# owkin/PyDESeq2

Measured on AMD Instinct MI355X. Metric: genes/sec end-to-end deseq2() (size factors->dispersion->IRLS->Wald), higher is better.
Workload: dtype f64

## Files before the change

### include/deseq_hip.h

```cpp
#ifndef DESEQ_HIP_H
#define DESEQ_HIP_H

#include <stddef.h>
#include <stdint.h>

#ifdef __cplusplus
extern "C" {
#endif

#define DSQ_ABI_VERSION 5
#define DSQ_MAX_P 128
#define DSQ_SHRINK_MAX_P 48
#define DSQ_BFGS_MAX_P 12

typedef struct dsq_ctx dsq_ctx;

enum dsq_status {
    DSQ_OK = 0,
    DSQ_ERR_HIP = -1,
    DSQ_ERR_ARG = -2,
    DSQ_ERR_RANGE = -3,
    DSQ_ERR_NOMEM = -4
};

// ... 114 lines not shown
                       const double* d_pinvXt, int ldx, int N, int G, int P, double min_disp, double max_disp,
                       double min_mu, double* d_normed_mean, double* d_mom, double* d_mu);
int dsq_dev_mom(dsq_ctx* ctx, const int32_t* d_y, int ldn, const double* d_sf, const double* d_Xt,
                const double* d_pinvXt, int ldx, int N, int G, int P, double min_disp,
                double max_disp, double* d_normed_mean, double* d_rough, double* d_moments,
                double* d_mom);
int dsq_dev_lin_mu(dsq_ctx* ctx, const int32_t* d_y, int ldn, const double* d_sf,
                   const double* d_Xt, const double* d_pinvXt, int ldx, int N, int G, int P,
                   double min_mu, double* d_mu);
int dsq_dev_alpha_mle(dsq_ctx* ctx, const int32_t* d_y, const double* d_mu, int ldn,
                      const double* d_Xt, int ldx, int N, int G, int P, const double* d_alpha_hat,
                      double min_disp, double max_disp, double prior_disp_var, int cr_reg,
                      int prior_reg, double* d_alpha, uint8_t* d_converged, int32_t* d_nfev,
                      double* d_nll_const, int const_mode);
typedef struct dsq_cells {
    const int32_t* d_cell_of;
    const double* d_Xc;
    const double* d_XX;
    int n_cells;
} dsq_cells;
int dsq_dev_mom_lin_coef(dsq_ctx* ctx, const int32_t* d_y, int ldn, const double* d_sf, const double* d_Xt,
                         const double* d_pinvXt, int ldx, int N, int G, int P, double min_disp, double max_disp,
                         double min_mu, double* d_normed_mean, double* d_mom, double* d_mu, double* d_coef);
int dsq_dev_alpha_mle2(dsq_ctx* ctx, const int32_t* d_y, const double* d_mu, int ldn, const double* d_Xt, int ldx,
                       int N, int G, int P, const double* d_alpha_hat, double min_disp, double max_disp,
                       double prior_disp_var, int cr_reg, int prior_reg, double* d_alpha, uint8_t* d_converged,
                       int32_t* d_nfev, double* d_nll_const, int const_mode, const dsq_cells* cells,
                       const double* d_coef, const double* d_sf, double min_mu);
int dsq_dev_alpha_mle3(dsq_ctx* ctx, const int32_t* d_y, const double* d_mu, int ldn, const double* d_Xt, int ldx,
                       int N, int G, int P, const double* d_alpha_hat, double min_disp, double max_disp,
                       double prior_disp_var, int cr_reg, int prior_reg, double* d_alpha, uint8_t* d_converged,
                       int32_t* d_nfev, double* d_nll_const, int const_mode, const dsq_cells* cells,
                       const double* d_coef, const double* d_sf, double min_mu, const int32_t* d_rows, int n_rows,
                       const int32_t* d_waves, int n_waves, const double* d_cell_mu);
typedef struct dsq_mix dsq_mix;
int dsq_mix_create(dsq_ctx* ctx, const double* design, int N, int P, dsq_mix** out);
void dsq_mix_destroy(dsq_mix* mix);
int dsq_mix_info(const dsq_mix* mix, int* n_slots, int* n_cells, int* n_continuous);
int dsq_mix_slots(const dsq_mix* mix, int32_t* h_slot_of);
int dsq_mix_bind(dsq_ctx* ctx, const uint16_t* d_ys, const uint8_t* d_big, const double* d_mu_slots);
int dsq_mix_bind2(dsq_ctx* ctx, const uint16_t* d_ys, const uint8_t* d_big, const double* d_mu_slots, int G);
int dsq_dev_mix_counts_to_slots(dsq_ctx* ctx, const int32_t* d_y, int ldn, int G, const dsq_mix* mix, uint16_t* d_ys,
                                uint8_t* d_big);
int dsq_dev_mix_mu_slots(dsq_ctx* ctx, const dsq_mix* mix, const double* d_beta, const double* d_sf, int G,
                         double* d_mu_slots);
int dsq_mix_takes_irls(const dsq_mix* mix, int full_rank);
int dsq_mix_launch_count(void);
int dsq_dev_alpha_mle4(dsq_ctx* ctx, const int32_t* d_y, const double* d_mu, int ldn, const double* d_Xt, int ldx,
                       int N, int G, int P, const double* d_alpha_hat, double min_disp, double max_disp,
                       double prior_disp_var, int cr_reg, int prior_reg, double* d_alpha, uint8_t* d_converged,
                       int32_t* d_nfev, double* d_nll_const, int const_mode, const dsq_cells* cells,
                       const double* d_coef, const double* d_sf, double min_mu, const int32_t* d_rows, int n_rows,
                       const int32_t* d_waves, int n_waves, const double* d_cell_mu, const dsq_mix* mix,
                       const double* d_beta);
int dsq_alpha_rows_eligible(int N, int P, int n_cells);
int dsq_alpha_needs_mu(int N, int P, int n_cells);
int dsq_dev_cell_mu(dsq_ctx* ctx, const double* d_beta, const dsq_cells* cells, int G, int P, double* d_cell_mu);
int dsq_dev_alpha_row_split(dsq_ctx* ctx, const int32_t* d_y, int ldn, int N, int G, int32_t* d_flags);
int dsq_dev_robust_disp(dsq_ctx* ctx, const int32_t* d_y, int ldn, const double* d_sf, const int32_t* d_cell_offsets,
                        const int32_t* d_cell_index, int n_cells, int whole, int max_cell, int N, int G,
                        double* d_robust_disp);
int dsq_dev_robust_disp2(dsq_ctx* ctx, const int32_t* d_y, int ldn, const double* d_sf, const int32_t* d_cell_offsets,
                         const int32_t* d_cell_index, int n_cells, int whole, int max_cell, int min_cell, int N, int G,
                         double* d_robust_disp);
int dsq_dev_lfc_fit(dsq_ctx* ctx, const int32_t* d_y, int ldn, const double* d_sf, const double* d_Xt,
                    const double* d_pinvXt, int ldx, int N, int G, int P, int full_rank, const double* d_disp,
                    double min_mu, double beta_tol, double min_beta, double max_beta, int maxiter, double* d_beta,
                    double* d_mu, double* d_hat, uint8_t* d_converged, int32_t* d_iters, const dsq_cells* cells,
                    const double* d_robust_disp, const uint8_t* d_flags, double cutoff, double* d_cooks,
                    uint8_t* d_any_all, uint8_t* d_any_use, uint8_t* d_any_use_nr, uint8_t* d_few_above,
                    const double* h_ridge, const double* h_contrast, double lfc_null, int alt, double* d_pvals,
                    double* d_stats, double* d_se);
int dsq_dev_lfc_fit2(dsq_ctx* ctx, const int32_t* d_y, int ldn, const double* d_sf, const double* d_Xt,
                     const double* d_pinvXt, int ldx, int N, int G, int P, int full_rank, const double* d_disp,
                     double min_mu, double beta_tol, double min_beta, double max_beta, int maxiter, double* d_beta,
                     double* d_mu, double* d_hat, uint8_t* d_converged, int32_t* d_iters, const dsq_cells* cells,
                     const double* d_robust_disp, const uint8_t* d_flags, double cutoff, double* d_cooks,
                     uint8_t* d_any_all, uint8_t* d_any_use, uint8_t* d_any_use_nr, uint8_t* d_few_above,
                     const double* h_ridge, const double* h_contrast, double lfc_null, int alt, double* d_pvals,
                     double* d_stats, double* d_se, const dsq_mix* mix, int cooks_ld);
int dsq_dev_replace_outliers2(dsq_ctx* ctx, const int32_t* d_y, const double* d_cooks, int ldn, const double* d_sf,
                              const uint8_t* d_flags, const int32_t* d_gene_idx, int n_sel, int N, double cutoff,
                              int32_t* d_y_out, uint8_t* d_all_zero, int cooks_ld, const dsq_mix* mix);
int dsq_dev_irls_layers(dsq_ctx* ctx, const int32_t* d_y, int ldn, const double* d_sf, const double* d_Xt, int ldx,
                        int N, int G, int P, const double* d_disp, const double* d_beta, double min_mu, double* d_mu,
                        double* d_hat);
int dsq_side_begin(dsq_ctx* ctx);
int dsq_side_end(dsq_ctx* ctx);
int dsq_side_wait(dsq_ctx* ctx);
int dsq_side_abort(dsq_ctx* ctx);
int dsq_dev_irls(dsq_ctx* ctx, const int32_t* d_y, int ldn, const double* d_sf, const double* d_Xt,
                 const double* d_pinvXt, int ldx, int N, int G, int P, int full_rank,
                 const double* d_disp, double min_mu, double beta_tol, double min_beta,
                 double max_beta, int maxiter, double* d_beta, double* d_mu, double* d_hat,
                 uint8_t* d_converged, int32_t* d_iters);
int dsq_dev_cooks(dsq_ctx* ctx, const int32_t* d_y, int ldn, const double* d_sf, const double* d_mu,
                  const double* d_hat, const int32_t* d_cell_offsets, const int32_t* d_cell_index,
                  int n_cells, int whole, int max_cell, const uint8_t* d_flags, int N, int G, int P,
                  double cutoff, double* d_cooks, double* d_robust_disp, uint8_t* d_any_all,
                  uint8_t* d_any_use, uint8_t* d_any_use_nr, uint8_t* d_few_above);
int dsq_dev_replace_outliers(dsq_ctx* ctx, const int32_t* d_y, const double* d_cooks, int ldn,
                             const double* d_sf, const uint8_t* d_flags, const int32_t* d_gene_idx,
                             int n_sel, int N, double cutoff, int32_t* d_y_out,
                             uint8_t* d_all_zero);
int dsq_dev_wald(dsq_ctx* ctx, const double* d_mu, int ldn, const double* d_sf, const double* d_Xt,
                 int ldx, int N, int G, int P, const double* d_disp, const double* d_beta,
                 const double* h_ridge, const double* h_contrast, double lfc_null, int alt,
                 double* d_pvals, double* d_stats, double* d_se);
int dsq_dev_lrt(dsq_ctx* ctx, const int32_t* d_y, int ldn, const double* d_sf, const double* d_Xt, int ldx, int P,
                const double* d_Xt_reduced, int ldx_reduced, int P_reduced, int N, int G, const double* d_disp,
                const double* d_beta, const double* d_beta_reduced, double* d_stats, double* d_pvals);
int dsq_dev_chisq_sf(dsq_ctx* ctx, const double* d_x, int n, int df, double* d_out);
int dsq_dev_trend_prior(dsq_ctx* ctx, const double* d_disp, const double* d_means, int n, double min_disp,
                        double max_disp, uint8_t* d_keep, double* d_fitted, double* d_work, double* h_coeffs2,
                        int* h_ok, int* h_n_outer, double* h_squared_logres);
int dsq_lfc_fork_begin(dsq_ctx* ctx);
int dsq_lfc_fork_end(dsq_ctx* ctx);
int dsq_lfc_set_part(dsq_ctx* ctx, const uint8_t* d_part, int want, int phase);
int dsq_lfc_takes_parts(int N, int P, const dsq_cells* cells, const dsq_mix* mix, int full_rank);
int dsq_dev_select_dispersions_part(dsq_ctx* ctx, double* d_genewise_raw, double* d_map_raw, const double* d_fitted, int n,
                                    double min_disp, double max_disp, double squared_logres, double* d_disp,
                                    uint8_t* d_outlier, uint8_t* d_map_converged, const uint8_t* d_conv_late, uint8_t* d_part,
                                    int mode, int ready_limit);
int dsq_alpha_set_late_flags(dsq_ctx* ctx, uint8_t* d_conv_late);
int dsq_lfc_prepare(dsq_ctx* ctx, const double* d_sf, int N, const double* h_ridge, const double* h_contrast, int P);
int dsq_dev_trend_eval(dsq_ctx* ctx, const double* d_normed_means, int n, double a0, double a1,
                       double* d_fitted);
int dsq_dev_select_dispersions(dsq_ctx* ctx, double* d_genewise_raw, double* d_map_raw,
                               const double* d_fitted, int n, double min_disp, double max_disp,
                               double squared_logres, double* d_disp, uint8_t* d_outlier);
int dsq_dev_scatter_rows_f64(dsq_ctx* ctx, const double* d_src, const int32_t* d_idx, int n_idx, int width,
                             double* d_dst);
int dsq_dev_mom_raw(dsq_ctx* ctx, const int32_t* d_y, int ldn, const double* d_ones, const double* d_sf,
                    const double* d_Xt, const double* d_pinvXt, int ldx, int N, int G, int P, double min_disp,
                    double max_disp, double* d_normed_mean, double* d_mom);
int dsq_dev_nll_const(dsq_ctx* ctx, const int32_t* d_y, int ldn, int N, int G, const double* d_disp, double* d_cst);
int dsq_dev_nll_scaled(dsq_ctx* ctx, const int32_t* d_y, const double* d_mu, int ldn, int N, int G,
                       const double* d_disp, const double* d_scale, const double* d_cst, double* d_nll);
int dsq_dev_logmeans_poscounts(dsq_ctx* ctx, const int32_t* d_y, int ldn, int N, int G, double* d_logmeans,
                               uint8_t* d_usable);
int dsq_dev_vst(dsq_ctx* ctx, const void* d_counts_sm, int count_type, int N, int G, const double* d_sf, int mode,
                double a0, double a1, double* d_out);
int dsq_inf_lfc_shrink_nbinom_glm2(dsq_ctx* ctx, const void* counts, int count_type, int count_layout,
                                   const double* design, const double* size, const double* offset, int N, int G,
                                   int P, double prior_no_shrink_scale, double prior_scale, int shrink_index,
                                   double* beta_out, double* inv_hessian_out, uint8_t* converged, int optimizer);
int dsq_inf_lfc_shrink_nbinom_glm(dsq_ctx* ctx, const void* counts, int count_type, int count_layout,
                                  const double* design, const double* size, const double* offset, int N, int G,
                                  int P, double prior_no_shrink_scale, double prior_scale, int shrink_index,
                                  double* beta_out, double* inv_hessian_out, uint8_t* converged);
int dsq_dev_lfc_shrink(dsq_ctx* ctx, const int32_t* d_y, int ldn, const double* d_offset, const double* d_Xt,
                       int ldx, int N, int G, int P, const double* d_size, double prior_no_shrink_scale,
                       double prior_scale, int shrink_index, double* d_beta, double* d_inv_hessian,
                       uint8_t* d_converged);
int dsq_dev_lfc_shrink2(dsq_ctx* ctx, const int32_t* d_y, int ldn, const double* d_offset, const double* d_Xt,
                        int ldx, int N, int G, int P, const double* d_size, double prior_no_shrink_scale,
                        double prior_scale, int shrink_index, double* d_beta, double* d_inv_hessian,
                        uint8_t* d_converged, double* d_ih_entry);
int dsq_dev_lfc_shrink3(dsq_ctx* ctx, const int32_t* d_y, int ldn, const double* d_offset, const double* d_Xt,
                        int ldx, int N, int G, int P, const double* d_size, double prior_no_shrink_scale,
                        double prior_scale, int shrink_index, double* d_beta, double* d_inv_hessian,
                        uint8_t* d_converged, double* d_ih_entry, int optimizer);
int dsq_dev_padj_prepare(dsq_ctx* ctx, const double* d_base_mean, const double* d_pvalue, int n, double alpha,
                         unsigned long long* d_sorted_p, int32_t* d_sorted_idx, uint8_t* d_bins,
                         double* h_out200, int* h_n_valid);
int dsq_dev_padj_finish(dsq_ctx* ctx, const unsigned long long* d_sorted_p, const int32_t* d_sorted_idx,
// ... 41 lines not shown
```

### pydeseq2_amd/_lib.py

```python
from __future__ import annotations

import ctypes as C
import os

import numpy as np

_HERE = os.path.dirname(os.path.abspath(__file__))
LIB_PATH = os.environ.get("DSQ_LIB", os.path.join(_HERE, "libdeseq_hip.so"))

DSQ_MAX_P = 128
DSQ_SHRINK_MAX_P = 48
_DEBUG = bool(os.environ.get("DSQ_DEBUG"))
SAMPLE_MAJOR, GENE_MAJOR = 0, 1
I32, I64 = 0, 1
ALT = {None: 0, "greaterAbs": 1, "lessAbs": 2, "greater": 3, "less": 4}

c_void_p, c_int, c_double, c_size_t = C.c_void_p, C.c_int, C.c_double, C.c_size_t
_vp = c_void_p
HOOK_FN = C.CFUNCTYPE(None, c_void_p)


class DsqCells(C.Structure):

    _fields_ = [("d_cell_of", C.c_void_p), ("d_Xc", C.c_void_p), ("d_XX", C.c_void_p), ("n_cells", C.c_int)]
# ... 89 lines not shown
    proto("dsq_dev_select_dispersions", _vp, _vp, _vp, _vp, c_int, c_double, c_double, c_double, _vp, _vp)
    proto("dsq_dev_scatter_rows_f64", _vp, _vp, _vp, c_int, c_int, _vp)
    proto("dsq_dev_sf_keys_compact", _vp, _vp, c_int, c_int, c_int, _vp, _vp, _vp, _vp, C.POINTER(c_int))
    proto("dsq_prior_mad_work_doubles", c_int, res=c_size_t)
    proto("dsq_size_factors_work_doubles", c_int, c_int, res=c_size_t)
    proto("dsq_dev_mom_lin_mu", _vp, _vp, c_int, _vp, _vp, _vp, c_int, c_int, c_int, c_int, c_double, c_double,
          c_double, _vp, _vp, _vp)
    proto("dsq_dev_mom_raw", _vp, _vp, c_int, _vp, _vp, _vp, _vp, c_int, c_int, c_int, c_int, c_double, c_double,
          _vp, _vp)
    proto("dsq_dev_nll_const", _vp, _vp, c_int, c_int, c_int, _vp, _vp)
    proto("dsq_dev_nll_scaled", _vp, _vp, _vp, c_int, c_int, c_int, _vp, _vp, _vp, _vp)
    proto("dsq_dev_logmeans_poscounts", _vp, _vp, c_int, c_int, c_int, _vp, _vp)
    proto("dsq_dev_vst", _vp, _vp, c_int, c_int, c_int, _vp, c_int, c_double, c_double, _vp)
    proto("dsq_inf_lfc_shrink_nbinom_glm2", _vp, _vp, c_int, c_int, _vp, _vp, _vp, c_int, c_int, c_int, c_double,
          c_double, c_int, _vp, _vp, _vp, c_int)
    proto("dsq_inf_lfc_shrink_nbinom_glm", _vp, _vp, c_int, c_int, _vp, _vp, _vp, c_int, c_int, c_int, c_double,
          c_double, c_int, _vp, _vp, _vp)
    proto("dsq_dev_lfc_shrink", _vp, _vp, c_int, _vp, _vp, c_int, c_int, c_int, c_int, _vp, c_double, c_double,
          c_int, _vp, _vp, _vp)
    proto("dsq_dev_lfc_shrink2", _vp, _vp, c_int, _vp, _vp, c_int, c_int, c_int, c_int, _vp, c_double, c_double,
          c_int, _vp, _vp, _vp, _vp)
    proto("dsq_dev_lfc_shrink3", _vp, _vp, c_int, _vp, _vp, c_int, c_int, c_int, c_int, _vp, c_double, c_double,
          c_int, _vp, _vp, _vp, _vp, c_int)
    proto("dsq_dev_padj_prepare", _vp, _vp, _vp, c_int, c_double, _vp, _vp, _vp, _vp, C.POINTER(c_int))
    proto("dsq_dev_padj_finish", _vp, _vp, _vp, _vp, c_int, c_int, c_int, _vp)
    proto("dsq_d2d", _vp, _vp, _vp, c_size_t)
    cells_p = C.POINTER(DsqCells)
    proto("dsq_dev_mom_lin_coef", _vp, _vp, c_int, _vp, _vp, _vp, c_int, c_int, c_int, c_int, c_double, c_double,
          c_double, _vp, _vp, _vp, _vp)
    proto("dsq_dev_alpha_mle2", _vp, _vp, _vp, c_int, _vp, c_int, c_int, c_int, c_int, _vp, c_double, c_double,
          c_double, c_int, c_int, _vp, _vp, _vp, _vp, c_int, cells_p, _vp, _vp, c_double)
    proto("dsq_dev_alpha_mle3", _vp, _vp, _vp, c_int, _vp, c_int, c_int, c_int, c_int, _vp, c_double, c_double,
          c_double, c_int, c_int, _vp, _vp, _vp, _vp, c_int, cells_p, _vp, _vp, c_double, _vp, c_int, _vp, c_int, _vp)
    proto("dsq_dev_alpha_mle4", _vp, _vp, _vp, c_int, _vp, c_int, c_int, c_int, c_int, _vp, c_double, c_double,
          c_double, c_int, c_int, _vp, _vp, _vp, _vp, c_int, cells_p, _vp, _vp, c_double, _vp, c_int, _vp, c_int, _vp,
          _vp, _vp)
    proto("dsq_mix_create", _vp, _vp, c_int, c_int, C.POINTER(_vp))
    proto("dsq_mix_destroy", _vp, res=None)
    proto("dsq_mix_launch_count")
    proto("dsq_mix_slots", _vp, _vp)
    proto("dsq_mix_takes_irls", _vp, c_int)
    proto("dsq_mix_info", _vp, C.POINTER(c_int), C.POINTER(c_int), C.POINTER(c_int))
    proto("dsq_alpha_rows_eligible", c_int, c_int, c_int)
    proto("dsq_alpha_needs_mu", c_int, c_int, c_int)
    proto("dsq_dev_cell_mu", _vp, _vp, cells_p, c_int, c_int, _vp)
    proto("dsq_dev_alpha_row_split", _vp, _vp, c_int, c_int, c_int, _vp)
    proto("dsq_dev_robust_disp", _vp, _vp, c_int, _vp, _vp, _vp, c_int, c_int, c_int, c_int, c_int, _vp)
    proto("dsq_dev_robust_disp2", _vp, _vp, c_int, _vp, _vp, _vp, c_int, c_int, c_int, c_int, c_int, c_int, _vp)
    proto("dsq_dev_lfc_fit", _vp, _vp, c_int, _vp, _vp, _vp, c_int, c_int, c_int, c_int, c_int, _vp, c_double,
          c_double, c_double, c_double, c_int, _vp, _vp, _vp, _vp, _vp, cells_p, _vp, _vp, c_double, _vp, _vp, _vp,
          _vp, _vp, _vp, _vp, c_double, c_int, _vp, _vp, _vp)
    proto("dsq_dev_lfc_fit2", _vp, _vp, c_int, _vp, _vp, _vp, c_int, c_int, c_int, c_int, c_int, _vp, c_double,
          c_double, c_double, c_double, c_int, _vp, _vp, _vp, _vp, _vp, cells_p, _vp, _vp, c_double, _vp, _vp, _vp,
          _vp, _vp, _vp, _vp, c_double, c_int, _vp, _vp, _vp, _vp, c_int)
    proto("dsq_dev_irls_layers", _vp, _vp, c_int, _vp, _vp, c_int, c_int, c_int, c_int, _vp, _vp, c_double, _vp, _vp)
    proto("dsq_side_begin", _vp)
    proto("dsq_side_end", _vp)
    proto("dsq_side_wait", _vp)
    proto("dsq_side_abort", _vp)
    proto("dsq_set_deferred", _vp, c_int)
    proto("dsq_lfc_fork_begin", _vp)
    proto("dsq_lfc_fork_end", _vp)
    proto("dsq_lfc_set_part", _vp, _vp, c_int, c_int)
    proto("dsq_lfc_takes_parts", c_int, c_int, cells_p, _vp, c_int)
    proto("dsq_dev_select_dispersions_part", _vp, _vp, _vp, _vp, c_int, c_double, c_double, c_double, _vp, _vp, _vp, _vp, _vp,
          c_int, c_int)
    proto("dsq_alpha_set_late_flags", _vp, _vp)
    proto("dsq_lfc_prepare", _vp, _vp, c_int, _vp, _vp, c_int)
    proto("dsq_irls_order_hint", _vp, _vp, c_int)
    proto("dsq_set_alpha_hook", _vp, _vp, _vp)
    proto("dsq_upload_counts_i32", _vp, _vp, c_int, c_size_t, _vp, C.POINTER(c_int))
    proto("dsq_host_alloc", _vp, c_size_t, C.POINTER(_vp))
    proto("dsq_host_free", _vp, _vp)
    proto("dsq_d2h_async", _vp, _vp, _vp, c_size_t)
    proto("dsq_h2d_async", _vp, _vp, _vp, c_size_t)
    proto("dsq_dev_alpha_mle", _vp, _vp, _vp, c_int, _vp, c_int, c_int, c_int, c_int, _vp, c_double,
          c_double, c_double, c_int, c_int, _vp, _vp, _vp, _vp, c_int)
    proto("dsq_dev_irls", _vp, _vp, c_int, _vp, _vp, _vp, c_int, c_int, c_int, c_int, c_int, _vp, c_double,
          c_double, c_double, c_double, c_int, _vp, _vp, _vp, _vp, _vp)
    proto("dsq_dev_cooks", _vp, _vp, c_int, _vp, _vp, _vp, _vp, _vp, c_int, c_int, c_int, _vp, c_int, c_int,
          c_int, c_double, _vp, _vp, _vp, _vp, _vp, _vp)
    proto("dsq_dev_replace_outliers", _vp, _vp, _vp, c_int, _vp, _vp, _vp, c_int, c_int, c_double, _vp, _vp)
    proto("dsq_dev_replace_outliers2", _vp, _vp, _vp, c_int, _vp, _vp, _vp, c_int, c_int, c_double, _vp, _vp, c_int, _vp)
    proto("dsq_dev_wald", _vp, _vp, c_int, _vp, _vp, c_int, c_int, c_int, c_int, _vp, _vp, _vp, _vp,
          c_double, c_int, _vp, _vp, _vp)
    proto("dsq_dev_lrt", _vp, _vp, c_int, _vp, _vp, c_int, c_int, _vp, c_int, c_int, c_int, c_int, _vp, _vp, _vp, _vp, _vp)
    proto("dsq_dev_chisq_sf", _vp, _vp, c_int, c_int, _vp)
    proto("dsq_dev_gather_rows_f64", _vp, _vp, c_int, _vp, c_int, c_int, _vp)
    proto("dsq_dev_gather_rows_i32", _vp, _vp, c_int, _vp, c_int, c_int, _vp)
    proto("dsq_comm_unique_id", _vp, C.c_char_p, c_int)
    proto("dsq_comm_init", _vp, C.c_char_p, c_int, c_int)
    proto("dsq_comm_destroy", _vp)
    proto("dsq_comm_allreduce_sum", _vp, _vp, c_size_t, c_int)
    proto("dsq_comm_allgather", _vp, _vp, _vp, c_size_t)
    proto("dsq_dev_sf_keys", _vp, _vp, c_int, c_int, c_int, _vp, _vp, _vp)
    proto("dsq_dev_sf_count", _vp, _vp, c_int, c_int, _vp)
    proto("dsq_dev_sf_init", _vp, _vp, c_int, _vp, _vp)
    proto("dsq_dev_sf_hist", _vp, _vp, c_int, c_int, _vp, c_int, _vp)
    proto("dsq_dev_sf_pick", _vp, _vp, c_int, c_int, _vp, _vp)
    proto("dsq_dev_sf_finish", _vp, _vp, _vp, c_int, _vp)
    _lib = lib
    return lib


EXPORTS = [
    "dsq_create", "dsq_destroy", "dsq_last_error", "dsq_device_info", "dsq_sync", "dsq_debug_pending_error", "dsq_timer_start",
    "dsq_timer_stop", "dsq_last_alpha_kernel", "dsq_malloc", "dsq_free", "dsq_memset", "dsq_h2d", "dsq_d2h", "dsq_h2d_2d",
    "dsq_d2h_2d", "dsq_inf_lin_reg_mu", "dsq_inf_irls", "dsq_inf_alpha_mle", "dsq_inf_wald_test",
    "dsq_inf_fit_rough_dispersions", "dsq_inf_fit_moments_dispersions", "dsq_dev_trend_loss_grad", "dsq_dev_trend_fit", "dsq_dev_prior_mad",
    "dsq_dev_counts_to_gene_major", "dsq_dev_f64_to_gene_major", "dsq_dev_logmeans",
    "dsq_dev_size_factors", "dsq_dev_mom", "dsq_dev_lin_mu", "dsq_dev_alpha_mle", "dsq_dev_irls",
    "dsq_dev_cooks", "dsq_dev_replace_outliers", "dsq_dev_wald", "dsq_dev_gather_rows_f64",
    "dsq_dev_gather_rows_i32", "dsq_comm_unique_id", "dsq_comm_init", "dsq_comm_destroy",
    "dsq_comm_allreduce_sum", "dsq_comm_allgather", "dsq_dev_sf_keys", "dsq_dev_sf_count", "dsq_dev_sf_init",
    "dsq_dev_sf_hist", "dsq_dev_sf_pick", "dsq_dev_sf_finish", "dsq_dev_trend_eval", "dsq_dev_trend_prior", "dsq_dev_select_dispersions",
    "dsq_dev_scatter_rows_f64", "dsq_d2d", "dsq_dev_mom_lin_mu", "dsq_dev_sf_keys_compact", "dsq_prior_mad_work_doubles", "dsq_size_factors_work_doubles", "dsq_dev_mom_raw", "dsq_dev_nll_const", "dsq_dev_nll_scaled", "dsq_dev_logmeans_poscounts", "dsq_dev_vst", "dsq_inf_lfc_shrink_nbinom_glm", "dsq_dev_lfc_shrink", "dsq_dev_lfc_shrink2", "dsq_dev_lfc_shrink3", "dsq_dev_padj_prepare", "dsq_dev_padj_finish", "dsq_host_alloc", "dsq_host_free", "dsq_d2h_async", "dsq_h2d_async",
    "dsq_dev_size_factors_new", "dsq_dev_mom_lin_coef", "dsq_dev_alpha_mle2", "dsq_dev_robust_disp", "dsq_dev_robust_disp2", "dsq_dev_lfc_fit", "dsq_dev_lfc_fit2", "dsq_dev_irls_layers",
    "dsq_side_begin", "dsq_side_end", "dsq_side_wait", "dsq_side_abort", "dsq_set_deferred", "dsq_irls_order_hint", "dsq_set_alpha_hook", "dsq_dev_alpha_mle3", "dsq_dev_alpha_mle4", "dsq_mix_create", "dsq_mix_destroy", "dsq_mix_info", "dsq_mix_slots", "dsq_mix_takes_irls", "dsq_dev_replace_outliers2", "dsq_mix_launch_count", "dsq_alpha_rows_eligible", "dsq_alpha_needs_mu", "dsq_dev_cell_mu", "dsq_dev_alpha_row_split",
    "dsq_upload_counts_i32", "dsq_inf_dispersion_trend_gamma_glm", "dsq_inf_grid_fit_alpha", "dsq_inf_grid_fit_beta",
    "dsq_inf_irls2", "dsq_inf_alpha_mle2", "dsq_inf_lfc_shrink_nbinom_glm2", "dsq_inf_fit_moments_dispersions2",
    "dsq_abi_version", "dsq_plugin_cache_config", "dsq_plugin_cache_clear", "dsq_plugin_cache_stats",
    "dsq_plugin_digest_host", "dsq_comm_info", "dsq_host_sync_count", "dsq_dev_pack2", "dsq_dev_unzip2",
    "dsq_mix_bind", "dsq_mix_bind2", "dsq_dev_mix_counts_to_slots", "dsq_dev_mix_mu_slots",
    "dsq_lfc_fork_begin", "dsq_lfc_fork_end", "dsq_lfc_set_part", "dsq_lfc_takes_parts", "dsq_dev_select_dispersions_part", "dsq_lfc_prepare", "dsq_alpha_set_late_flags",
    "dsq_dev_lrt", "dsq_dev_chisq_sf",
]


def ptr(a):
    if a is None:
        return None
    if isinstance(a, np.ndarray):
        return a.ctypes.data
    return a


class Context:

    def __init__(self, device: int = 0):
        self.lib = load()
        h = _vp()
        rc = self.lib.dsq_create(int(device), C.byref(h))
        if rc != 0 or not h.value:
            raise DsqError(
                f"dsq_create(device={device}) failed (rc={rc}): no usable MI355X / HIP runtime. "
                "pydeseq2_amd runs on the GPU only."
            )
        self.h = h
        self.device = device

    def close(self):
        if getattr(self, "h", None) is not None and self.h.value:
            for bufs in self.__dict__.pop("_padj_buffers", {}).values():
                for b in bufs:
                    b.free()
            self.lib.dsq_destroy(self.h)
            self.h = _vp()

    def __del__(self):
        try:
            self.close()
        except Exception:
            pass

    def call(self, name, *args):
        rc = getattr(self.lib, name)(self.h, *args)
        if _DEBUG:
            pend = self.lib.dsq_debug_pending_error().decode()
            if pend:
                print(f"[dsq debug] pending HIP error after {name}: {pend}", flush=True)
        if rc != 0:
            msg = self.lib.dsq_last_error(self.h).decode(errors="replace")
            if rc == -2:
                raise ValueError(msg)
            raise DsqError(f"{name} failed (rc={rc}): {msg}")

    def device_info(self):
        name, arch = C.create_string_buffer(256), C.create_string_buffer(256)
        cu, mem = c_int(), c_size_t()
        self.call("dsq_device_info", name, 256, C.byref(cu), C.byref(mem), arch, 256)
        return dict(name=name.value.decode(), arch=arch.value.decode(), cu_count=cu.value, mem_bytes=mem.value)

    def sync(self):
        self.call("dsq_sync")

    def timer_start(self):
        self.call("dsq_timer_start")

    def timer_stop(self) -> float:
        ms = C.c_float()
        self.call("dsq_timer_stop", C.byref(ms))
        return float(ms.value)

    def malloc(self, nbytes: int) -> int:
        p = _vp()
        self.call("dsq_malloc", c_size_t(int(nbytes)), C.byref(p))
        return p.value

    def free(self, dptr):
        if dptr:
            self.call("dsq_free", _vp(dptr))

    def memset(self, dptr, value, nbytes):
        self.call("dsq_memset", _vp(dptr), int(value), c_size_t(int(nbytes)))

    def h2d(self, dptr, arr: np.ndarray):
        arr = np.ascontiguousarray(arr)
        self.call("dsq_h2d", _vp(dptr), _vp(arr.ctypes.data), c_size_t(arr.nbytes))
# ... 116 lines not shown
```

### pydeseq2_amd/csrc/dsq_capi_dev.hip

```cpp
#include "dsq_capi_internal.h"

extern "C" {

int dsq_dev_counts_to_gene_major(dsq_ctx* ctx, const void* d_src, int count_type, int layout, int N, int G,
                                 int32_t* d_dst, int ldn, int* h_bad) {
    DSQ_CHECK_ARG(ldn >= N, "ldn < N");
    int* d_bad = (int*)ctx->d_scratch;
    DSQ_HIP(hipMemsetAsync(d_bad, 0, sizeof(int), ctx->stream));
    DSQ_HIP(dsq::launch_transpose_counts(ctx->stream, d_src, count_type, layout, N, G, d_dst, ldn, d_bad));
    if (h_bad) {
        DSQ_HIP(hipMemcpyAsync(h_bad, d_bad, sizeof(int), hipMemcpyDeviceToHost, ctx->stream));
        DSQ_HIP(hipStreamSynchronize(ctx->stream));
    }
    return DSQ_OK;
}

int dsq_dev_f64_to_gene_major(dsq_ctx* ctx, const double* d_src, int layout, int N, int G, double* d_dst,
                              int ldn) {
    DSQ_HIP(dsq::launch_transpose_f64(ctx->stream, d_src, layout, N, G, d_dst, ldn));
    return DSQ_OK;
}

int dsq_dev_logmeans(dsq_ctx* ctx, const int32_t* d_y, int ldn, int N, int G, double* d_logmeans,
                     uint8_t* d_nonzero) {
// ... 442 lines not shown
                     const double* d_pinvXt, int ldx, int N, int G, int P, int full_rank, const double* d_disp,
                     double min_mu, double beta_tol, double min_beta, double max_beta, int maxiter, double* d_beta,
                     double* d_mu, double* d_hat, uint8_t* d_converged, int32_t* d_iters, const dsq_cells* cells,
                     const double* d_robust_disp, const uint8_t* d_flags, double cutoff, double* d_cooks,
                     uint8_t* d_any_all, uint8_t* d_any_use, uint8_t* d_any_use_nr, uint8_t* d_few_above,
                     const double* h_ridge, const double* h_contrast, double lfc_null, int alt, double* d_pvals,
                     double* d_stats, double* d_se, const dsq_mix* mix, int cooks_ld) {
    DSQ_CHECK_ARG(P >= 1 && P <= DSQ_MAX_P, "P out of range");
    DSQ_CHECK_ARG(mix == nullptr || (mix->d.P == P && mix->d.N == N), "mix: built for another design");
    DSQ_CHECK_ARG(cooks_ld == 0 || (mix != nullptr && cooks_ld >= mix->d.Ns && dsq::irls_takes_mix(&mix->d, full_rank)),
                  "cooks_ld: a slot-ordered Cook's layer needs a mixed design the kernel takes and a pitch >= its slots");
    DSQ_CHECK_ARG(cells == nullptr || cells->n_cells <= dsq::kMaxCells, "too many design cells for the cell path");
    DSQ_CHECK_ARG(d_flags == nullptr || (d_robust_disp && d_any_all && d_any_use && d_any_use_nr && d_few_above),
                  "the fused Cook's bookkeeping needs the robust dispersions and the four flag vectors");
    DSQ_CHECK_ARG(h_ridge == nullptr || (h_contrast && d_pvals && d_stats && d_se && alt >= 0 && alt <= 4),
                  "the fused Wald test needs contrast, outputs and a valid alternative");
    if (G <= 0) return DSQ_OK;
    dsq::IrlsExtras ex{};
    ex.cells = to_cells(cells);
    if (mix != nullptr) ex.mix = &mix->d;
    ex.cooks_ld = cooks_ld;
    if (d_flags != nullptr) {
        ex.robust_disp = d_robust_disp; ex.flags = d_flags; ex.cutoff = cutoff; ex.cooks = d_cooks;
        ex.any_all = d_any_all; ex.any_use = d_any_use; ex.any_use_nr = d_any_use_nr; ex.few_above = d_few_above;
    }
    if (h_ridge != nullptr) {
        double* d_ridge;
        double* h_stage;
        { const int rc = ridge_stage(ctx, P, &d_ridge, &h_stage); if (rc != DSQ_OK) return fail(ctx, rc, "ridge staging: out of memory"); }
        double* d_contrast = d_ridge + P * P;
        const bool in_place = ctx->lfc_part != nullptr &&
                              (ctx->lfc_phase == 2 || (ctx->lfc_phase == 1 && ctx->lfc_prepared_wald &&
                                                       ctx->lfc_prepared_N == N && ctx->lfc_prepared_P == P));
        if (!in_place) {
            std::memcpy(h_stage, h_ridge, (size_t)P * P * sizeof(double));
            std::memcpy(h_stage + P * P, h_contrast, (size_t)P * sizeof(double));
            DSQ_HIP(hipMemcpyAsync(d_ridge, h_stage, (size_t)(P * P + P) * sizeof(double), hipMemcpyHostToDevice,
                                   ctx->stream));
        }
        ex.ridge = d_ridge; ex.contrast = d_contrast; ex.lfc_null = lfc_null; ex.alt = alt;
        ex.pvals = d_pvals; ex.stats = d_stats; ex.se = d_se;
    }
    return run_irls(ctx, d_y, ldn, d_sf, d_Xt, d_pinvXt, ldx, N, G, P, full_rank, d_disp, min_mu, beta_tol, min_beta,
                    max_beta, maxiter, d_beta, d_mu, d_hat, d_converged, d_iters, &ex);
}

int dsq_dev_lfc_fit(dsq_ctx* ctx, const int32_t* d_y, int ldn, const double* d_sf, const double* d_Xt,
                    const double* d_pinvXt, int ldx, int N, int G, int P, int full_rank, const double* d_disp,
                    double min_mu, double beta_tol, double min_beta, double max_beta, int maxiter, double* d_beta,
                    double* d_mu, double* d_hat, uint8_t* d_converged, int32_t* d_iters, const dsq_cells* cells,
                    const double* d_robust_disp, const uint8_t* d_flags, double cutoff, double* d_cooks,
                    uint8_t* d_any_all, uint8_t* d_any_use, uint8_t* d_any_use_nr, uint8_t* d_few_above,
                    const double* h_ridge, const double* h_contrast, double lfc_null, int alt, double* d_pvals,
                    double* d_stats, double* d_se) {
    return dsq_dev_lfc_fit2(ctx, d_y, ldn, d_sf, d_Xt, d_pinvXt, ldx, N, G, P, full_rank, d_disp, min_mu, beta_tol,
                            min_beta, max_beta, maxiter, d_beta, d_mu, d_hat, d_converged, d_iters, cells, d_robust_disp,
                            d_flags, cutoff, d_cooks, d_any_all, d_any_use, d_any_use_nr, d_few_above, h_ridge, h_contrast,
                            lfc_null, alt, d_pvals, d_stats, d_se, nullptr, 0);
}

int dsq_dev_cooks(dsq_ctx* ctx, const int32_t* d_y, int ldn, const double* d_sf, const double* d_mu,
                  const double* d_hat, const int32_t* d_cell_offsets, const int32_t* d_cell_index,
                  int n_cells, int whole, int max_cell, const uint8_t* d_flags, int N, int G, int P,
                  double cutoff, double* d_cooks, double* d_robust_disp, uint8_t* d_any_all,
                  uint8_t* d_any_use, uint8_t* d_any_use_nr, uint8_t* d_few_above) {
    DSQ_CHECK_ARG((whole ? N : max_cell) <= 16384, "a design cell with more than 16384 samples is not supported");
    DSQ_HIP(dsq::launch_cooks(ctx->stream, d_y, ldn, d_sf, d_mu, d_hat, d_cell_offsets, d_cell_index,
                              n_cells, whole, max_cell, d_flags, N, G, P, cutoff, d_cooks, d_robust_disp,
                              d_any_all, d_any_use, d_any_use_nr, d_few_above));
    return DSQ_OK;
}

int dsq_dev_replace_outliers2(dsq_ctx* ctx, const int32_t* d_y, const double* d_cooks, int ldn,
                              const double* d_sf, const uint8_t* d_flags, const int32_t* d_gene_idx,
                              int n_sel, int N, double cutoff, int32_t* d_y_out, uint8_t* d_all_zero, int cooks_ld,
                              const dsq_mix* mix) {
    DSQ_CHECK_ARG(cooks_ld == 0 || (mix != nullptr && mix->d.N == N && cooks_ld >= mix->d.Ns),
                  "cooks_ld: a slot-ordered Cook's layer comes with the mixed design that wrote it");
    DSQ_HIP(dsq::launch_replace(ctx->stream, d_y, d_cooks, ldn, d_sf, d_flags, d_gene_idx, n_sel, N, cutoff,
                                d_y_out, d_all_zero, cooks_ld, cooks_ld != 0 ? mix->d.slot_of : nullptr));
    return DSQ_OK;
}

int dsq_dev_replace_outliers(dsq_ctx* ctx, const int32_t* d_y, const double* d_cooks, int ldn,
                             const double* d_sf, const uint8_t* d_flags, const int32_t* d_gene_idx,
                             int n_sel, int N, double cutoff, int32_t* d_y_out, uint8_t* d_all_zero) {
    return dsq_dev_replace_outliers2(ctx, d_y, d_cooks, ldn, d_sf, d_flags, d_gene_idx, n_sel, N, cutoff, d_y_out,
                                     d_all_zero, 0, nullptr);
}

int dsq_dev_wald(dsq_ctx* ctx, const double* d_mu, int ldn, const double* d_sf, const double* d_Xt, int ldx,
                 int N, int G, int P, const double* d_disp, const double* d_beta, const double* h_ridge,
                 const double* h_contrast, double lfc_null, int alt, double* d_pvals, double* d_stats,
                 double* d_se) {
    DSQ_CHECK_ARG(P >= 1 && P <= DSQ_MAX_P, "P out of range");
    DSQ_CHECK_ARG(alt >= 0 && alt <= 4, "unknown alternative hypothesis");
    double* d_ridge;
    double* h_unused;
    { const int rc = ridge_stage(ctx, P, &d_ridge, &h_unused); if (rc != DSQ_OK) return fail(ctx, rc, "ridge staging: out of memory"); }
    double* d_contrast = d_ridge + (P <= 48 ? 48 * 48 : P * P);
    DSQ_HIP(hipMemcpyAsync(d_ridge, h_ridge, (size_t)P * P * sizeof(double), hipMemcpyHostToDevice, ctx->stream));
    DSQ_HIP(hipMemcpyAsync(d_contrast, h_contrast, (size_t)P * sizeof(double), hipMemcpyHostToDevice, ctx->stream));
    DSQ_HIP(hipStreamSynchronize(ctx->stream));
    DSQ_HIP(dsq::launch_wald(ctx->stream, d_mu, ldn, d_sf, d_Xt, ldx, N, G, P, d_disp, d_beta, d_ridge,
                             d_contrast, lfc_null, alt, d_pvals, d_stats, d_se));
    return DSQ_OK;
}

int dsq_dev_lrt(dsq_ctx* ctx, const int32_t* d_y, int ldn, const double* d_sf, const double* d_Xt, int ldx, int P,
                const double* d_Xt_reduced, int ldx_reduced, int P_reduced, int N, int G, const double* d_disp,
                const double* d_beta, const double* d_beta_reduced, double* d_stats, double* d_pvals) {
    DSQ_CHECK_ARG(P >= 2 && P <= DSQ_MAX_P, "P out of range");
    DSQ_CHECK_ARG(P_reduced >= 1 && P_reduced < P, "P_reduced: between 1 and P - 1 columns");
    DSQ_CHECK_ARG(ldn >= N && ldx >= N && ldx_reduced >= N, "a leading dimension is smaller than N");
    DSQ_HIP(dsq::launch_lrt(ctx->stream, d_y, ldn, d_sf, d_Xt, ldx, P, d_Xt_reduced, ldx_reduced, P_reduced, N, G, d_disp,
                            d_beta, d_beta_reduced, d_stats, d_pvals));
    return DSQ_OK;
}

int dsq_dev_chisq_sf(dsq_ctx* ctx, const double* d_x, int n, int df, double* d_out) {
    DSQ_CHECK_ARG(df >= 1 && df <= DSQ_MAX_P - 1, "df: an integer between 1 and 127");
    DSQ_HIP(dsq::launch_chisq_sf(ctx->stream, d_x, n, df, d_out));
    return DSQ_OK;
}

int dsq_dev_gather_rows_f64(dsq_ctx* ctx, const double* d_src, int ld, const int32_t* d_idx, int n_idx,
                            int ncols, double* d_dst) {
    DSQ_HIP(dsq::launch_gather_rows_f64(ctx->stream, d_src, ld, d_idx, n_idx, ncols, d_dst));
    return DSQ_OK;
}

int dsq_dev_lfc_shrink3(dsq_ctx* ctx, const int32_t* d_y, int ldn, const double* d_offset, const double* d_Xt,
                        int ldx, int N, int G, int P, const double* d_size, double prior_no_shrink_scale,
                        double prior_scale, int shrink_index, double* d_beta, double* d_inv_hessian,
                        uint8_t* d_converged, double* d_ih_entry, int optimizer) {
    DSQ_CHECK_ARG(P >= 1 && P <= DSQ_SHRINK_MAX_P, "P out of range (apeGLM shrinkage: at most 48 design columns)");
    DSQ_CHECK_ARG(shrink_index >= 0 && shrink_index < P, "shrink_index out of range");
    DSQ_CHECK_ARG(d_ih_entry == nullptr || P <= DSQ_BFGS_MAX_P, "d_ih_entry: designs of at most 12 columns (wider: d_inv_hessian)");
    DSQ_CHECK_ARG(optimizer >= 0 && optimizer <= 2, "optimizer: 0 (L-BFGS-B), 1 (BFGS) or 2 (Newton-CG)");
    DSQ_CHECK_ARG(optimizer == 0 || P <= DSQ_BFGS_MAX_P, "optimizer BFGS / Newton-CG: designs of at most 12 columns");
    DSQ_HIP(dsq::launch_shrink(ctx->stream, d_y, ldn, d_offset, d_Xt, ldx, N, G, P, d_size, prior_no_shrink_scale,
                               prior_scale, shrink_index, d_beta, d_inv_hessian, d_converged, d_ih_entry, optimizer));
    return DSQ_OK;
}

int dsq_dev_lfc_shrink2(dsq_ctx* ctx, const int32_t* d_y, int ldn, const double* d_offset, const double* d_Xt,
                        int ldx, int N, int G, int P, const double* d_size, double prior_no_shrink_scale,
                        double prior_scale, int shrink_index, double* d_beta, double* d_inv_hessian,
                        uint8_t* d_converged, double* d_ih_entry) {
    return dsq_dev_lfc_shrink3(ctx, d_y, ldn, d_offset, d_Xt, ldx, N, G, P, d_size, prior_no_shrink_scale, prior_scale,
                               shrink_index, d_beta, d_inv_hessian, d_converged, d_ih_entry, 0);
}

int dsq_dev_lfc_shrink(dsq_ctx* ctx, const int32_t* d_y, int ldn, const double* d_offset, const double* d_Xt,
                       int ldx, int N, int G, int P, const double* d_size, double prior_no_shrink_scale,
                       double prior_scale, int shrink_index, double* d_beta, double* d_inv_hessian,
                       uint8_t* d_converged) {
    return dsq_dev_lfc_shrink2(ctx, d_y, ldn, d_offset, d_Xt, ldx, N, G, P, d_size, prior_no_shrink_scale, prior_scale,
                               shrink_index, d_beta, d_inv_hessian, d_converged, nullptr);
}

int dsq_dev_vst(dsq_ctx* ctx, const void* d_counts_sm, int count_type, int N, int G, const double* d_sf, int mode,
                double a0, double a1, double* d_out) {
    DSQ_CHECK_ARG(mode == 0 || mode == 1, "mode: 0 parametric trend, 1 mean dispersion");
    DSQ_HIP(dsq::launch_vst(ctx->stream, d_counts_sm, count_type, N, G, d_sf, mode, a0, a1, d_out));
    return DSQ_OK;
// ... 222 lines not shown
```

### pydeseq2_amd/csrc/dsq_capi_internal.h

```cpp
#pragma once
#include <hip/hip_runtime.h>

#include <dlfcn.h>

#include <algorithm>
#include <cmath>
#include <cstdio>
#include <cstdlib>
#include <cstring>
#include <string>
#include <thread>
#include <vector>

#include <atomic>
#include <mutex>

extern std::atomic<unsigned long long> g_dsq_host_syncs;
#define hipStreamSynchronize(s) (++g_dsq_host_syncs, (hipStreamSynchronize)(s))
#define hipEventSynchronize(e) (++g_dsq_host_syncs, (hipEventSynchronize)(e))

#include "../../include/deseq_hip.h"
#include "dsq_launch.h"
namespace dsq_pc {
struct Cache;
}

struct dsq_mix {
    dsq::MixDesign d{};
    void* d_block = nullptr;
    int device = 0;
};

struct dsq_ctx {
    int device = 0;
    hipStream_t stream = nullptr;
    hipStream_t main_stream = nullptr, side_stream = nullptr;
    hipStream_t small_stream = nullptr;
    hipEvent_t ev_small0 = nullptr, ev_small1 = nullptr;
    hipEvent_t ev_fork = nullptr, ev_join = nullptr;
    hipEvent_t ev0 = nullptr, ev1 = nullptr, evk0 = nullptr, evk1 = nullptr;
    float last_kernel_ms = 0.0f;
    int last_n_grid = 0;
    double* d_scratch = nullptr;
    int32_t* d_counter = nullptr;
    int32_t* d_list = nullptr;
    size_t list_cap = 0;
    void* d_trend_grid = nullptr;
    double* d_lsf = nullptr;
    void* d_sum = nullptr;
    size_t sum_cap = 0, sum_sort_bytes = 0;
    size_t lsf_cap = 0;
    void* stage[2] = {nullptr, nullptr};
    hipEvent_t stage_ev[2] = {nullptr, nullptr};
    void* d_stage16[2] = {nullptr, nullptr};
    const int32_t* d_irls_hint = nullptr;
    int irls_hint_genes = 0;
    void (*alpha_hook)(void*) = nullptr;
    void* alpha_hook_arg = nullptr;
    int deferred = 0;
    int32_t* h_pin = nullptr;
    double* d_ridge_wide = nullptr;
    double* h_ridge_wide = nullptr;
    void* d_ws = nullptr;
    size_t ws_cap = 0;
    void* d_resume = nullptr;
    size_t resume_cap = 0;
    void* d_mix = nullptr;
    size_t mix_cap = 0;
    const uint16_t* bind_ys = nullptr;
    const uint8_t* bind_big = nullptr;
    const double* bind_mu = nullptr;
    int bind_G = 0;
    void* d_mixw = nullptr;
    size_t mixw_cap = 0;
    int32_t* d_redo = nullptr;
    size_t redo_cap = 0;
    hipStream_t lfc_stream = nullptr, lfc_return = nullptr;
    hipEvent_t ev_lfc_fork = nullptr, ev_lfc_done = nullptr, ev_lfc_part = nullptr;
    const uint8_t* lfc_part = nullptr;
    int lfc_want = 0, lfc_phase = 0;
    uint8_t* alpha_conv_late = nullptr;
    int lfc_prepared_N = 0, lfc_prepared_P = 0, lfc_prepared_wald = 0;
    int lfc_pending_G = 0;
    int32_t* d_lfc_aux = nullptr;
    size_t lfc_aux_cap = 0;
    dsq_pc::Cache* pc = nullptr;
    struct PluginDesign* designs = nullptr;
    void* comm = nullptr;
    int comm_rank = 0, comm_world = 1;
    std::string err;
};

void dsq_internal_destroy_plugin(dsq_ctx* ctx);

namespace {
void fire_alpha_hook(void* c) {
    dsq_ctx* ctx = (dsq_ctx*)c;
    if (ctx->alpha_hook == nullptr) return;
    void (*fn)(void*) = ctx->alpha_hook;
    ctx->alpha_hook = nullptr;
    fn(ctx->alpha_hook_arg);
}
}

namespace {

constexpr size_t kScratchBytes = 32 * 1024;
constexpr int kDeferredMaxGenes = 2048;

inline int ridge_stage(dsq_ctx* ctx, int P, double** d, double** h) {
    if (P <= 48) {
        *d = ctx->d_scratch + 1664;
        *h = (double*)(ctx->h_pin + (P <= 32 ? 16 : 4096));
        return DSQ_OK;
    }
    const size_t bytes = (size_t)(DSQ_MAX_P * DSQ_MAX_P + DSQ_MAX_P) * sizeof(double);
    if (ctx->d_ridge_wide == nullptr && hipMalloc((void**)&ctx->d_ridge_wide, bytes) != hipSuccess) {
        ctx->d_ridge_wide = nullptr;
        return DSQ_ERR_NOMEM;
    }
    if (ctx->h_ridge_wide == nullptr && hipHostMalloc((void**)&ctx->h_ridge_wide, bytes, hipHostMallocDefault) != hipSuccess) {
        ctx->h_ridge_wide = nullptr;
        return DSQ_ERR_NOMEM;
    }
    *d = ctx->d_ridge_wide;
    *h = ctx->h_ridge_wide;
    return DSQ_OK;
}

int fail(dsq_ctx* c, int code, const std::string& msg) {
    if (c) {
        c->err = msg;
        c->bind_ys = nullptr;
        c->bind_big = nullptr;
        c->bind_mu = nullptr;
        c->bind_G = 0;
    }
    return code;
}

#define DSQ_HIP(call)                                                                            \
    do {                                                                                         \
        hipError_t e_ = (call);                                                                  \
        if (e_ != hipSuccess)                                                                    \
            return fail(ctx, DSQ_ERR_HIP, std::string(#call) + ": " + hipGetErrorString(e_));    \
    } while (0)

#define DSQ_CHECK_ARG(cond, msg)                          \
    do {                                                  \
        if (!(cond)) return fail(ctx, DSQ_ERR_ARG, msg);  \
    } while (0)

inline int pad16(int n) { return (n + 15) & ~15; }

hipError_t ensure_list(dsq_ctx* c, size_t n) {
    if (n <= c->list_cap) return hipSuccess;
    if (c->d_list) (void)hipFree(c->d_list);
    c->d_list = nullptr;
    c->list_cap = 0;
    hipError_t e = hipMalloc((void**)&c->d_list, n * sizeof(int32_t));
    if (e == hipSuccess) c->list_cap = n;
    return e;
}
// ... 150 lines not shown
                                  prior_var, cr_reg, prior_reg, d_alpha, d_conv, d_nfev, d_cnt, ctx->d_list,
                                  d_nll_const, const_mode, extras, d_cnt + 1));
    }
    DSQ_HIP(hipEventRecord(ctx->evk1, ctx->stream));
    fire_alpha_hook(ctx);
    int32_t* h_cnt = ctx->h_pin + 1;
    const bool deferred = ctx->deferred && G <= kDeferredMaxGenes && optimizer == 0 &&
                          !dsq::alpha_is_wide(P, extras != nullptr ? extras->cells.C : 0);
    const int32_t* n_dev = deferred ? d_cnt : nullptr;
    int32_t n_grid = G;
    if (!deferred) {
        DSQ_HIP(hipMemcpyAsync(h_cnt, d_cnt, sizeof(int32_t), hipMemcpyDeviceToHost, ctx->stream));
        DSQ_HIP(hipStreamSynchronize(ctx->stream));
        DSQ_HIP(hipEventElapsedTime(&ctx->last_kernel_ms, ctx->evk0, ctx->evk1));
        n_grid = *h_cnt;
        ctx->last_n_grid = n_grid;
    } else {
        ctx->last_kernel_ms = -1.0f;
        ctx->last_n_grid = -1;
    }
    if (n_grid > 0) {
        auto up = [](size_t b) { return (b + 255) & ~(size_t)255; };
        const bool from_cells = extras != nullptr && extras->cell_mu != nullptr;
        const bool from_beta = extras != nullptr && extras->mix_beta != nullptr && d_mu == nullptr;
        const bool rebuild = extras != nullptr && (extras->coef != nullptr || from_cells || from_beta);
        const size_t b_work = up((size_t)n_grid * dsq::kAlphaGridWorkDoubles * sizeof(double));
        const size_t b_mu = rebuild ? up((size_t)n_grid * ldn * sizeof(double)) : 0;
        const size_t b_idx = rebuild ? up((size_t)n_grid * sizeof(int32_t)) : 0;
        DSQ_HIP(ensure_ws(ctx, b_work + b_mu + b_idx));
        char* w = (char*)ctx->d_ws;
        double* work = (double*)w;
        if (rebuild) {
            double* musub = (double*)(w + b_work);
            int32_t* idx = (int32_t*)(w + b_work + b_mu);
            if (from_beta)
                DSQ_HIP(dsq::launch_mu_from_beta(ctx->stream, extras->mix_beta, extras->sf, d_Xt, ldx, N, P, ctx->d_list,
                                                 n_grid, musub, ldn, idx, n_dev));
            else if (from_cells)
                DSQ_HIP(dsq::launch_mu_from_cells(ctx->stream, extras->cell_mu, extras->cells.C, extras->sf,
                                                  extras->cells.cell_of, N, ctx->d_list, n_grid, musub, ldn, idx, n_dev));
            else
                DSQ_HIP(dsq::launch_mu_from_coef(ctx->stream, extras->coef, extras->sf, d_Xt, ldx, N, P, extras->min_mu,
                                                 ctx->d_list, n_grid, musub, ldn, idx, n_dev));
            DSQ_HIP(dsq::launch_alpha_grid(ctx->stream, d_y, musub, ldn, d_Xt, ldx, N, P, min_disp, max_disp, d_alpha,
                                           ctx->d_list, n_grid, work, n_dev, true));
        } else {
            DSQ_HIP(dsq::launch_alpha_grid(ctx->stream, d_y, d_mu, ldn, d_Xt, ldx, N, P, min_disp, max_disp, d_alpha,
                                           ctx->d_list, n_grid, work, n_dev));
        }
    }
    return DSQ_OK;
}

}


namespace {
constexpr int kIrlsOrderMinGenes = 1024;
bool irls_order_enabled() {
    static const bool v = getenv("DSQ_NO_IRLS_ORDER") == nullptr;
    return v;
}
}

namespace {
int run_irls(dsq_ctx* ctx, const int32_t* d_y, int ldn, const double* d_sf, const double* d_Xt,
             const double* d_pinvXt, int ldx, int N, int G, int P, int full_rank, const double* d_disp,
             double min_mu, double beta_tol, double min_beta, double max_beta, int maxiter,
             double* d_beta, double* d_mu, double* d_hat, uint8_t* d_converged, int32_t* d_iters,
             const dsq::IrlsExtras* extras, int optimizer = 0) {
    if (G <= 0) return DSQ_OK;
    DSQ_CHECK_ARG(optimizer == 0 || optimizer == 1, "optimizer: 0 (L-BFGS-B) or 1 (BFGS)");
    struct Unbind {
        dsq_ctx* c;
        ~Unbind() { c->bind_ys = nullptr; c->bind_big = nullptr; c->bind_mu = nullptr; c->bind_G = 0; }
    } unbind{ctx};
    if (ctx->bind_G != 0 && ctx->bind_G != G) {
        ctx->bind_ys = nullptr; ctx->bind_big = nullptr; ctx->bind_mu = nullptr; ctx->bind_G = 0;
    }
    dsq::IrlsExtras ex_local{};
    if (extras != nullptr) ex_local = *extras;
    const dsq::MixDesign* const extras_in_mix = ex_local.mix;
    ex_local.optimizer = optimizer;
    DSQ_CHECK_ARG(optimizer == 0 || P <= DSQ_BFGS_MAX_P, "optimizer=\"BFGS\": designs of at most 12 columns");
    extras = &ex_local;
    const uint8_t* const part = ctx->lfc_part;
    const int part_want = ctx->lfc_want, phase = part != nullptr ? ctx->lfc_phase : 0;
    ctx->lfc_part = nullptr; ctx->lfc_phase = 0;
    if (phase != 0) {
        DSQ_CHECK_ARG(phase == 1 || phase == 2, "dsq_lfc_set_part: phase 1 or 2");
        DSQ_CHECK_ARG(optimizer == 0 && !ctx->deferred &&
                          dsq::irls_takes_parts(N, P, ex_local.cells.C, ex_local.mix, full_rank),
                      "a fit in two launches: the default rescue optimiser, not deferred, a design the part-aware kernels take");
        DSQ_CHECK_ARG(phase == 1 ? ctx->lfc_pending_G == 0 : ctx->lfc_pending_G == G,
                      "a fit in two launches: phase 2 follows the phase 1 of the same genes");
        ex_local.part = part;
        ex_local.part_want = part_want;
        ex_local.part_shared_ready = phase == 2 ? 1 : 0;
    }
    const bool ordered = G >= kIrlsOrderMinGenes && dsq::irls_takes_rows(N, P, ex_local.cells.C) && irls_order_enabled();
    const size_t list_ints = (size_t)G * (ordered ? 2 : 1) + (ordered ? (size_t)dsq::irls_order_work_ints() : 0);
    int32_t* fb_list = nullptr;
    int32_t* fb_count = ctx->d_counter;
    if (phase == 1) {
        if (list_ints > ctx->lfc_aux_cap) {
            if (ctx->d_lfc_aux) (void)hipFree(ctx->d_lfc_aux);
            ctx->d_lfc_aux = nullptr; ctx->lfc_aux_cap = 0;
            DSQ_HIP(hipMalloc((void**)&ctx->d_lfc_aux, list_ints * sizeof(int32_t)));
            ctx->lfc_aux_cap = list_ints;
        }
        fb_list = ctx->d_lfc_aux;
        fb_count = ctx->d_counter + 8;
    } else {
        DSQ_HIP(ensure_list(ctx, list_ints));
        fb_list = ctx->d_list;
    }
    if (ordered) {
        int32_t* d_order = fb_list + G;
        DSQ_HIP(dsq::launch_irls_order(ctx->stream, d_disp, ctx->irls_hint_genes == G ? ctx->d_irls_hint : nullptr, G,
                                       d_order, d_order + G));
        ex_local.order = d_order;
    }
    ctx->d_irls_hint = nullptr; ctx->irls_hint_genes = 0;
    const bool prepared = phase == 1 && ctx->lfc_prepared_N == N && ctx->lfc_prepared_P == P;
    ctx->lfc_prepared_N = 0; ctx->lfc_prepared_P = 0; ctx->lfc_prepared_wald = 0;
    if (phase != 2 && !prepared) {
        if ((size_t)N > ctx->lsf_cap) {
            if (ctx->d_lsf) (void)hipFree(ctx->d_lsf);
            ctx->d_lsf = nullptr; ctx->lsf_cap = 0;
            DSQ_HIP(hipMalloc((void**)&ctx->d_lsf, (size_t)N * sizeof(double)));
            ctx->lsf_cap = (size_t)N;
        }
        DSQ_HIP(dsq::launch_log_vec(ctx->stream, d_sf, N, ctx->d_lsf));
    }
    if (!prepared) DSQ_HIP(hipMemsetAsync(fb_count, 0, 2 * sizeof(int32_t), ctx->stream));
    if (ex_local.mix != nullptr && dsq::irls_takes_mix(ex_local.mix, full_rank)) {
        const int n_layers = ((ex_local.flags != nullptr && ex_local.cooks != nullptr) ? 1 : 0) + (d_mu != nullptr ? 1 : 0) +
                             (d_hat != nullptr ? 1 : 0);
        const size_t need = dsq::irls_mix_work_bytes(*ex_local.mix, G, n_layers);
        if (need > ctx->mixw_cap) {
            if (ctx->d_mixw) (void)hipFree(ctx->d_mixw);
            ctx->d_mixw = nullptr; ctx->mixw_cap = 0;
            DSQ_HIP(hipMalloc(&ctx->d_mixw, need));
            ctx->mixw_cap = need;
        }
        ex_local.mix_work = ctx->d_mixw;
        ex_local.mix_work_bytes = ctx->mixw_cap;
        ex_local.mix_queue = fb_count + 1;
        ex_local.mix_ys = ctx->bind_ys;
        ex_local.mix_big = ctx->bind_big;
        if (ex_local.mix_ys == nullptr || ex_local.mix_big == nullptr) {
            const size_t Ns = (size_t)ex_local.mix->Ns;
            const size_t need_s = (size_t)G * Ns * sizeof(uint16_t) + (size_t)G + 256;
            if (need_s > ctx->mix_cap) {
                if (ctx->d_mix) (void)hipFree(ctx->d_mix);
                ctx->d_mix = nullptr; ctx->mix_cap = 0;
                DSQ_HIP(hipMalloc(&ctx->d_mix, need_s));
                ctx->mix_cap = need_s;
            }
            uint16_t* t = (uint16_t*)ctx->d_mix;
            DSQ_HIP(dsq::launch_mix_counts_to_slots(ctx->stream, d_y, ldn, *ex_local.mix, G, t, (uint8_t*)(t + (size_t)G * Ns)));
            ex_local.mix_ys = t;
            ex_local.mix_big = (const uint8_t*)(t + (size_t)G * Ns);
        }
    } else {
        ex_local.mix = nullptr;
// ... 50 lines not shown
```

### pydeseq2_amd/csrc/dsq_k_irls.hip

```cpp
#include <type_traits>

#include "dsq_dispatch.h"
#include "dsq_irls.h"
#include "dsq_launch.h"

namespace dsq {

#if defined(DSQ_PHASE_TIMING)
__device__ unsigned long long g_phase_total_irls[16];
#endif

#ifndef DSQ_IRLS_WAVES_P2
#define DSQ_IRLS_WAVES_P2 4
#endif
constexpr int irls_min_waves(int p) { return p <= 2 ? DSQ_IRLS_WAVES_P2 : (p <= 5 ? 1 : 2); }

template <int P>
__device__ __forceinline__ void epilogue_begin(LfcEpilogue& E, const IrlsExtras& ex, int g, int ldn) {
    if (ex.flags != nullptr) {
        E.flags = ex.flags; E.robust_disp = ex.robust_disp[g]; E.cutoff = ex.cutoff;
        E.cooks_row = ex.cooks ? ex.cooks + (size_t)g * ldn : nullptr;
    }
    if (ex.ridge != nullptr) { E.ridge = ex.ridge; E.contrast = ex.contrast; E.lfc_null = ex.lfc_null; E.alt = ex.alt; }
}
// ... 9 lines not shown

template <int P, int CELL>
__global__ __launch_bounds__(kBlock, CELL == 1 ? cell_min_waves(P) : irls_min_waves(P)) void k_irls(const int32_t* __restrict__ y, int ldn,
                                                 const double* __restrict__ sf, const double* __restrict__ lsf,
                                                 const double* __restrict__ Xt,
                                                 const double* __restrict__ pinvXt, int ldx, int N,
                                                 int G, int full_rank, const double* __restrict__ disp,
                                                 double min_mu, double beta_tol, double min_beta,
                                                 double max_beta, int maxiter, double* __restrict__ beta,
                                                 double* __restrict__ mu, double* __restrict__ hat,
                                                 uint8_t* __restrict__ conv, int32_t* __restrict__ iters,
                                                 int32_t* __restrict__ fb_count,
                                                 int32_t* __restrict__ fb_list, IrlsExtras ex, int stage) {
    __shared__ typename std::conditional<CELL == 1, CellWork<P>, char>::type cellw[kWavesPerBlock];
    extern __shared__ __attribute__((aligned(16))) double irls_lds[];
    const int w = threadIdx.x >> 6;
    const int g = blockIdx.x * kWavesPerBlock + w;
    if (ex.part != nullptr) {
        bool any = false;
#pragma unroll
        for (int k = 0; k < kWavesPerBlock; ++k) {
            const int gk = blockIdx.x * kWavesPerBlock + k;
            any = any || (gk < G && ex.part[gk] == (uint8_t)ex.part_want);
        }
        if (!any) return;
    }
    log_tab_fill();
    double* lds_next = irls_lds;
    if (CELL) {
        constexpr int T = Tri<P>::N;
        double* sXX = lds_next;
        double* sXc = sXX + ex.cells.C * T;
        lds_next = sXc + ex.cells.C * P;
        for (int i = threadIdx.x; i < ex.cells.C * T; i += kBlock) sXX[i] = ex.cells.XX[i];
        for (int i = threadIdx.x; i < ex.cells.C * P; i += kBlock) sXc[i] = ex.cells.Xc[i];
        ex.cells.XX = sXX;
        ex.cells.Xc = sXc;
    }
    const int32_t* yrow = y + (size_t)(g < G ? g : G - 1) * ldn;
    if (stage) {
        const int npad = (N + 15) & ~15;
        double* s_sf = lds_next;
        double* s_lsf = s_sf + npad;
        int32_t* s_cell = (int32_t*)(s_lsf + npad);
        int32_t* s_y = s_cell + npad + (size_t)w * npad;
        for (int n = threadIdx.x; n < N; n += kBlock) {
            s_sf[n] = sf[n];
            s_lsf[n] = lsf != nullptr ? lsf[n] : 0.0;
            if (CELL) s_cell[n] = ex.cells.cell_of[n];
        }
        for (int n = threadIdx.x & 63; n < N; n += 64) s_y[n] = yrow[n];
        sf = s_sf;
        if (lsf != nullptr) lsf = s_lsf;
        if (CELL) ex.cells.cell_of = s_cell;
        yrow = s_y;
    }
    __syncthreads();
    if (g >= G) return;
    if (ex.part != nullptr && ex.part[g] != (uint8_t)ex.part_want) return;
#if defined(DSQ_PHASE_TIMING)
    if ((threadIdx.x & 63) == 0) {
        for (int k = 0; k < kPhases; ++k) g_ph_acc[w][k] = 0;
        g_ph_last[w] = clock64();
        g_ph_cur[w] = 0;
    }
#endif
    IrlsArgs A;
    A.y = yrow; A.sf = sf; A.lsf = lsf; A.Xt = Xt; A.pinvXt = pinvXt; A.ldx = ldx; A.N = N;
    A.disp = disp[g]; A.min_mu = min_mu; A.beta_tol = beta_tol; A.min_beta = min_beta;
    A.max_beta = max_beta; A.maxiter = maxiter; A.full_rank = full_rank != 0;
    if (CELL) { A.cells = &ex.cells; A.cell_ws = CELL == 1 ? (void*)&cellw[w] : nullptr; }
    LfcEpilogue E;
    epilogue_begin<P>(E, ex, g, ldn);
    double b[P];
    const IrlsOut o = irls_gene<DeviceWave, P, CELL>(A, b, mu ? mu + (size_t)g * ldn : nullptr,
                                                     hat ? hat + (size_t)g * ldn : nullptr, &E);
    if ((threadIdx.x & 63) == 0) {
#pragma unroll
        for (int j = 0; j < P; ++j) beta[(size_t)g * P + j] = b[j];
        conv[g] = (uint8_t)o.converged;
        if (iters != nullptr) iters[g] = o.iters;
        if (o.fallback) fb_list[atomicAdd(fb_count, 1)] = g;
        else epilogue_store(E, ex, g);
    }
#if defined(DSQ_PHASE_TIMING)
    DSQ_PHASE(0);
    if ((threadIdx.x & 63) == 0)
        for (int k = 0; k < kPhases; ++k) atomicAdd(&g_phase_total_irls[k], (unsigned long long)g_ph_acc[w][k]);
#endif
}

constexpr int kRowGenes = kBlock / 16;
template <int P>
__global__ __launch_bounds__(kBlock, 2) void k_irls_row(const int32_t* __restrict__ y, int ldn,
                                                        const double* __restrict__ sf, const double* __restrict__ lsf,
                                                        const double* __restrict__ Xt,
                                                        const double* __restrict__ pinvXt, int ldx, int N, int G,
                                                        int full_rank, const double* __restrict__ disp, double min_mu,
                                                        double beta_tol, double min_beta, double max_beta, int maxiter,
                                                        double* __restrict__ beta, double* __restrict__ mu,
                                                        double* __restrict__ hat, uint8_t* __restrict__ conv,
                                                        int32_t* __restrict__ iters, int32_t* __restrict__ fb_count,
                                                        int32_t* __restrict__ fb_list, IrlsExtras ex) {
    __shared__ CellWork<P> cellw[kRowGenes];
    extern __shared__ __attribute__((aligned(16))) double irls_lds[];
    constexpr int T = Tri<P>::N;
    const int row = threadIdx.x >> 4;
    const int slot = blockIdx.x * kRowGenes + row;
    int g = slot < G ? (ex.order != nullptr ? ex.order[slot] : slot) : G;
    if (ex.part != nullptr && g < G && ex.part[g] != (uint8_t)ex.part_want) g = G;
    if (ex.part != nullptr && __syncthreads_count(g < G) == 0) return;
    log_tab_fill();
    double* sXX = irls_lds;
    double* sXc = sXX + ex.cells.C * T;
    const int npad = (N + 15) & ~15;
    double* s_sf = sXc + ex.cells.C * P;
    double* s_lsf = s_sf + npad;
    double* s_pinvc = s_lsf + npad;
    int32_t* s_cell = (int32_t*)(s_pinvc + ex.cells.C * P);
    int32_t* s_rep = s_cell + npad;
    for (int i = threadIdx.x; i < ex.cells.C * T; i += kBlock) sXX[i] = ex.cells.XX[i];
    for (int i = threadIdx.x; i < ex.cells.C * P; i += kBlock) sXc[i] = ex.cells.Xc[i];
    if (full_rank) {
        for (int i = threadIdx.x; i < ex.cells.C; i += kBlock) s_rep[i] = 0x7fffffff;
        __syncthreads();
    }
    for (int n = threadIdx.x; n < N; n += kBlock) {
        s_sf[n] = sf[n];
        s_lsf[n] = lsf != nullptr ? lsf[n] : 0.0;
        const int c = ex.cells.cell_of[n];
        s_cell[n] = c;
        if (full_rank) atomicMin(&s_rep[c], n);
    }
    if (full_rank) {
        __syncthreads();
        for (int i = threadIdx.x; i < ex.cells.C * P; i += kBlock) s_pinvc[i] = pinvXt[(i % P) * ldx + s_rep[i / P]];
    }
    ex.cells.XX = sXX;
    ex.cells.Xc = sXc;
    ex.cells.cell_of = s_cell;
    __syncthreads();
    if (g >= G) return;
    IrlsArgs A;
    A.y = y + (size_t)g * ldn; A.sf = s_sf; A.lsf = lsf != nullptr ? s_lsf : nullptr; A.Xt = Xt; A.pinvXt = pinvXt;
    A.ldx = ldx; A.N = N;
    A.disp = disp[g]; A.min_mu = min_mu; A.beta_tol = beta_tol; A.min_beta = min_beta;
    A.max_beta = max_beta; A.maxiter = maxiter; A.full_rank = full_rank != 0;
    A.cells = &ex.cells;
    A.cell_ws = (void*)&cellw[row];
    A.pinvc = full_rank ? s_pinvc : nullptr;
#if defined(DSQ_PHASE_TIMING)
    if ((threadIdx.x & 63) == 0) {
        for (int k = 0; k < kPhases; ++k) g_ph_acc[threadIdx.x >> 6][k] = 0;
        g_ph_last[threadIdx.x >> 6] = clock64();
        g_ph_cur[threadIdx.x >> 6] = 0;
    }
#endif
    LfcEpilogue E;
    epilogue_begin<P>(E, ex, g, ldn);
    double b[P];
    const IrlsOut o = irls_gene<RowWave, P, 1>(A, b, mu ? mu + (size_t)g * ldn : nullptr,
                                               hat ? hat + (size_t)g * ldn : nullptr, &E);
    if ((threadIdx.x & 15) == 0) {
#pragma unroll
        for (int j = 0; j < P; ++j) beta[(size_t)g * P + j] = b[j];
        conv[g] = (uint8_t)o.converged;
// ... 100 lines not shown
    const int g = fb_list[k];
    IrlsArgs A;
    A.y = y + (size_t)g * ldn; A.sf = sf; A.lsf = lsf; A.Xt = Xt; A.pinvXt = pinvXt; A.ldx = ldx; A.N = N;
    A.disp = disp[g]; A.min_mu = min_mu; A.beta_tol = beta_tol; A.min_beta = min_beta;
    A.max_beta = max_beta; A.maxiter = maxiter; A.full_rank = full_rank != 0;
    __shared__ IrlsRescueWork<P> work[kWavesPerBlock];
    LfcEpilogue E;
    epilogue_begin<P>(E, ex, g, ldn);
    if (ex.cooks_ld != 0 && E.cooks_row != nullptr) E.cooks_row = ex.cooks_tmp + (size_t)k * ldn;
    double b[P];
    const IrlsOut o = irls_rescue_gene<DeviceWave, P>(A, work[threadIdx.x >> 6], b,
                                                      mu ? mu + (size_t)g * ldn : nullptr,
                                                      hat ? hat + (size_t)g * ldn : nullptr, &E, ex.optimizer);
    if ((threadIdx.x & 63) == 0) {
#pragma unroll
        for (int j = 0; j < P; ++j) beta[(size_t)g * P + j] = b[j];
        conv[g] = (uint8_t)o.converged;
        if (iters != nullptr) iters[g] = o.iters;
        epilogue_store(E, ex, g);
    }
}

__global__ __launch_bounds__(kBlock) void k_grid_beta(const int32_t* __restrict__ y, int ldn,
                                                      const double* __restrict__ sf, const double* __restrict__ Xt,
                                                      int ldx, int N, int G, const double* __restrict__ disp,
                                                      double min_mu, double min_beta, double max_beta, int grid_length,
                                                      double* __restrict__ beta) {
    const int g = blockIdx.x * kWavesPerBlock + (threadIdx.x >> 6);
    if (g >= G) return;
    IrlsArgs A;
    A.y = y + (size_t)g * ldn; A.sf = sf; A.lsf = nullptr; A.Xt = Xt; A.pinvXt = nullptr; A.ldx = ldx; A.N = N;
    A.disp = disp[g]; A.min_mu = min_mu; A.beta_tol = 0.0; A.min_beta = min_beta; A.max_beta = max_beta;
    A.maxiter = 0; A.full_rank = false;
    const double a = 1.0 / A.disp;
    double c = 0.0;
    for (int n = DeviceWave::lane(); n < N; n += 64) {
        const double yv = (double)A.y[n];
        c += lgamma_pos(yv + a) - lgamma_pos(yv + 1.0);
    }
    const double cst = DeviceWave::sum(c) - N * lgamma_pos(a);
    double b[2];
    grid_fit_beta2<DeviceWave>(A, a, cst, b, grid_length);
    if ((threadIdx.x & 63) == 0) { beta[2 * g] = b[0]; beta[2 * g + 1] = b[1]; }
}

hipError_t launch_grid_beta(hipStream_t st, const int32_t* y, int ldn, const double* sf, const double* Xt, int ldx,
                            int N, int G, const double* disp, double min_mu, double min_beta, double max_beta,
                            int grid_length, double* beta) {
    if (G <= 0) return hipSuccess;
    hipLaunchKernelGGL(k_grid_beta, dim3(genes_to_blocks(G)), dim3(kBlock), 0, st, y, ldn, sf, Xt, ldx, N, G, disp,
                       min_mu, min_beta, max_beta, grid_length, beta);
    return hipGetLastError();
}

template <int P>
__global__ __launch_bounds__(kBlock) void k_irls_layers(const int32_t* __restrict__ y, int ldn,
                                                        const double* __restrict__ sf, const double* __restrict__ Xt,
                                                        int ldx, int N, int G, const double* __restrict__ disp,
                                                        const double* __restrict__ beta, double min_mu,
                                                        double* __restrict__ mu, double* __restrict__ hat) {
    log_tab_fill();
    __syncthreads();
    const int g = blockIdx.x * kWavesPerBlock + (threadIdx.x >> 6);
    if (g >= G) return;
    IrlsArgs A;
    A.y = y + (size_t)g * ldn; A.sf = sf; A.lsf = nullptr; A.Xt = Xt; A.pinvXt = nullptr; A.ldx = ldx; A.N = N;
    A.disp = disp[g]; A.min_mu = min_mu; A.beta_tol = 0.0; A.min_beta = 0.0; A.max_beta = 0.0; A.maxiter = 0;
    A.full_rank = false;
    double b[P], M[Tri<P>::N], r[P], S;
#pragma unroll
    for (int j = 0; j < P; ++j) b[j] = beta[(size_t)g * P + j];
    irls_sweep<DeviceWave, P>(A, b, 1.0 / A.disp, S, M, r);
    irls_finish<DeviceWave, P>(A, b, M, mu ? mu + (size_t)g * ldn : nullptr, hat ? hat + (size_t)g * ldn : nullptr);
}

hipError_t launch_irls_layers(hipStream_t st, const int32_t* y, int ldn, const double* sf, const double* Xt, int ldx,
                              int N, int G, int P_, const double* disp, const double* beta, double min_mu, double* mu,
                              double* hat) {
    if (G <= 0) return hipSuccess;
    if (P_ > DSQ_REG_MAX_P)
        return launch_wide_irls_layers(st, y, ldn, sf, Xt, ldx, N, G, P_, disp, beta, min_mu, mu, hat);
    DSQ_DISPATCH_P(P_, hipLaunchKernelGGL(k_irls_layers<P>, dim3(genes_to_blocks(G)), dim3(kBlock), 0, st, y, ldn, sf,
                                          Xt, ldx, N, G, disp, beta, min_mu, mu, hat))
    return hipGetLastError();
}

constexpr int kRowMinP = 3;
static bool row_wave_enabled() {
    static const bool v = getenv("DSQ_NO_ROW_WAVE") == nullptr;
    return v;
}
static int row_min_p() {
    static const int v = getenv("DSQ_ROW_MIN_P") ? atoi(getenv("DSQ_ROW_MIN_P")) : 5;
    return v;
}
static size_t row_lds_bytes(int C, int P, int N) {
    const int npad = (N + 15) & ~15;
    return (size_t)C * (P * (P + 1) / 2 + 2 * P) * sizeof(double) + (size_t)npad * 20 + (size_t)kMaxCells * 4;
}

static int irls_row_min_genes() {
    const char* e = getenv("DSQ_IRLS_ROW_MIN_G");
    return e ? atoi(e) : 1024;
}

bool irls_takes_parts(int N, int P_, int n_cells, const MixDesign* mix, int full_rank) {
    (void)N;
    if (mix != nullptr && irls_takes_mix(mix, full_rank)) return true;
    return !(P_ > DSQ_REG_MAX_P || (P_ >= wide_min_p() && (n_cells == 0 || wide_with_cells())));
}

bool irls_takes_rows(int N, int P_, int n_cells) {
    if (P_ > DSQ_REG_MAX_P || (P_ >= wide_min_p() && (n_cells == 0 || wide_with_cells()))) return false;
    return n_cells > kSmallCells && P_ >= kRowMinP && P_ >= row_min_p() && row_wave_enabled() &&
           row_lds_bytes(n_cells, P_, N) <= 40 * 1024;
}

#define DSQ_MIXI_DECL(Q_)                                                                                             \
    bool irls_mix_fits_q##Q_(int Ns, int P);                                                                          \
    void irls_mix_grid_q##Q_(int Ns, int P, int G, int* blocks, int* nw);                                             \
    hipError_t launch_irls_mix_q##Q_(hipStream_t, const int32_t*, int, const uint16_t*, const uint8_t*, const MixDesign&, \
                                     const double*, int, int32_t*, const double*, double, double, double, int, double*, \
                                     double*, double*, uint8_t*, int32_t*, int32_t*, int32_t*, const IrlsExtras&, void*, \
                                     size_t);
DSQ_MIXI_DECL(1)
DSQ_MIXI_DECL(2)
DSQ_MIXI_DECL(3)
#undef DSQ_MIXI_DECL

bool irls_takes_mix(const MixDesign* mix, int full_rank) {
    static const bool off = getenv("DSQ_NO_IRLS_MIX") != nullptr;
    if (off || mix == nullptr || !full_rank || mix->Ginv == nullptr || !alpha_mix_enabled()) return false;
    switch (mix->Q) {
        case 1: return irls_mix_fits_q1(mix->Ns, mix->P);
        case 2: return irls_mix_fits_q2(mix->Ns, mix->P);
        case 3: return irls_mix_fits_q3(mix->Ns, mix->P);
        default: return false;
    }
}

size_t irls_mix_work_bytes(const MixDesign& D, int G, int n_layers) {
    int blocks = 0, nw = 0;
    if (D.Q == 1) irls_mix_grid_q1(D.Ns, D.P, G, &blocks, &nw);
    else if (D.Q == 2) irls_mix_grid_q2(D.Ns, D.P, G, &blocks, &nw);
    else if (D.Q == 3) irls_mix_grid_q3(D.Ns, D.P, G, &blocks, &nw);
    (void)blocks; (void)nw; (void)n_layers;
    return (((size_t)D.Ns * 17 + 63) & ~(size_t)63) + (size_t)(G > 0 ? G : 0) * (kMixMaxP * (kMixMaxP + 1) / 2) * sizeof(double) + 64;
}

static hipError_t launch_irls_mix(hipStream_t st, const int32_t* y, int ldn, const MixDesign& D, const double* sf, int G,
                                  int32_t* queue, const double* disp, double min_mu, double beta_tol, double max_beta,
                                  int maxiter, double* beta, double* mu, double* hat, uint8_t* conv, int32_t* iters,
                                  int32_t* fb_count, int32_t* fb_list, const IrlsExtras& ex, void* work,
                                  size_t work_bytes) {
    switch (D.Q) {
        case 1: return launch_irls_mix_q1(st, y, ldn, ex.mix_ys, ex.mix_big, D, sf, G, queue, disp, min_mu, beta_tol, max_beta, maxiter, beta, mu,
                                          hat, conv, iters, fb_count, fb_list, ex, work, work_bytes);
        case 2: return launch_irls_mix_q2(st, y, ldn, ex.mix_ys, ex.mix_big, D, sf, G, queue, disp, min_mu, beta_tol, max_beta, maxiter, beta, mu,
                                          hat, conv, iters, fb_count, fb_list, ex, work, work_bytes);
        case 3: return launch_irls_mix_q3(st, y, ldn, ex.mix_ys, ex.mix_big, D, sf, G, queue, disp, min_mu, beta_tol, max_beta, maxiter, beta, mu,
                                          hat, conv, iters, fb_count, fb_list, ex, work, work_bytes);
        default: return hipErrorInvalidValue;
    }
}

hipError_t launch_irls(hipStream_t st, const int32_t* y, int ldn, const double* sf, const double* lsf,
// ... 127 lines not shown
```

### pydeseq2_amd/csrc/dsq_k_stats.hip

```cpp
#include <cfloat>
#include <hip/hip_cooperative_groups.h>

#include <cstdio>

#include "dsq_dispatch.h"
#include "dsq_launch.h"
#include "dsq_stats.h"
#include "dsq_trend.h"

namespace dsq {

struct LdsSorter {
    __device__ __forceinline__ static void wave_sync() {
        __builtin_amdgcn_fence(__ATOMIC_RELEASE, "wavefront");
        __builtin_amdgcn_wave_barrier();
        __builtin_amdgcn_fence(__ATOMIC_ACQUIRE, "wavefront");
    }
    __device__ __forceinline__ int operator()(double* buf, int n) const {
        int L = 1;
        while (L < n) L <<= 1;
        const int lane = threadIdx.x & 63;
        for (int k = n + lane; k < L; k += 64) buf[k] = INFINITY;
        wave_sync();
        for (int k = 2; k <= L; k <<= 1) {
// ... 1049 lines not shown
                                                               const double* __restrict__ sf,
                                                               const int32_t* __restrict__ cell_offsets,
                                                               const int32_t* __restrict__ cell_index, int n_cells,
                                                               int whole, int N, int G,
                                                               double* __restrict__ robust_disp,
                                                               int32_t* __restrict__ redo_count,
                                                               int32_t* __restrict__ redo_list, int can_redo) {
    __shared__ BucketWork W[WPB];
    const int w = threadIdx.x >> 6;
    const int g = blockIdx.x * WPB + w;
    if (g >= G) return;
    CellPlan C{cell_offsets, cell_index, n_cells, whole};
    bool failed;
    const double ar = robust_disp_gene_lean<DeviceWave>(y + (size_t)g * ldn, sf, C, N, W[w], failed);
    if ((threadIdx.x & 63) == 0) {
        if (failed && can_redo) redo_list[atomicAdd(redo_count, 1)] = g;
        else robust_disp[g] = failed ? NAN : ar;
    }
}

bool robust_disp_lean_eligible(int min_cell, int max_cell, int whole, int N) {
    const bool off = getenv("DSQ_NO_ROBUST_LEAN") != nullptr;
    const char* mn = getenv("DSQ_ROBUST_LEAN_MIN");
    const int min_big = mn != nullptr ? atoi(mn) : 2048;
    return !off && (whole ? N : min_cell) >= kTrimBucketMin && (whole ? N : max_cell) >= min_big;
}

hipError_t launch_robust_disp(hipStream_t st, const int32_t* y, int ldn, const double* sf,
                              const int32_t* cell_offsets, const int32_t* cell_index, int n_cells, int whole,
                              int max_cell, int N, int G, double* robust_disp, int min_cell, int32_t* redo) {
    if (G <= 0) return hipSuccess;
    const int biggest = whole ? N : max_cell;
    static const bool seg_off = getenv("DSQ_NO_SEG_CELLS") != nullptr;
    const int seg_len = (!whole && !seg_off && biggest <= kSegMaxCell) ? next_pow2(biggest < 2 ? 2 : biggest) : 0;
    const int cap = seg_len > 0 ? kSegBatch + kSegBatch / 2 : trim_cap(biggest);
    const int stride = cap + trim_work_doubles(biggest);
    const size_t per_wave = (size_t)stride * sizeof(double);
    const bool big = biggest >= kTrimBucketMin;
    const bool buffered_fits = per_wave <= 160 * 1024;
    if (!buffered_fits && redo == nullptr) return hipErrorInvalidValue;
    const bool lean = redo != nullptr && (!buffered_fits || robust_disp_lean_eligible(min_cell, max_cell, whole, N));
    if (lean) {
        hipError_t e = hipMemsetAsync(redo, 0, sizeof(int32_t), st);
        if (e != hipSuccess) return e;
        constexpr int WPB = 4;
        hipLaunchKernelGGL((k_robust_disp_lean<WPB>), dim3((G + WPB - 1) / WPB), dim3(64 * WPB), 0, st, y, ldn, sf,
                           cell_offsets, cell_index, n_cells, whole, N, G, robust_disp, redo, redo + 1,
                           buffered_fits ? 1 : 0);
        e = hipGetLastError();
        if (e != hipSuccess || !buffered_fits) return e;
    }
    const int32_t* list = lean ? redo + 1 : nullptr;
    const int32_t* n_dev = lean ? redo : nullptr;
#define DSQ_RD_LAUNCH(WPB) \
    do { if (big) DSQ_RD_LAUNCH_(WPB, true); else DSQ_RD_LAUNCH_(WPB, false); } while (0)
#define DSQ_RD_LAUNCH_(WPB, BIG)                                                                             \
    do {                                                                                                     \
        if (per_wave * WPB > 48 * 1024) {                                                                    \
            (void)hipFuncSetAttribute((const void*)k_robust_disp<WPB, BIG>, hipFuncAttributeMaxDynamicSharedMemorySize, \
                                      (int)(per_wave * WPB));                                                \
            (void)hipGetLastError();                                                                         \
        }                                                                                                    \
        hipLaunchKernelGGL((k_robust_disp<WPB, BIG>), dim3((G + WPB - 1) / WPB), dim3(64 * WPB), per_wave * WPB, st, y, \
                           ldn, sf, cell_offsets, cell_index, n_cells, whole, cap, stride, seg_len, N, G, robust_disp, \
                           list, n_dev);                                                                     \
    } while (0)
    if (per_wave * 4 <= 64 * 1024) DSQ_RD_LAUNCH(4);
    else if (per_wave * 2 <= 160 * 1024) DSQ_RD_LAUNCH(2);
    else DSQ_RD_LAUNCH(1);
#undef DSQ_RD_LAUNCH
#undef DSQ_RD_LAUNCH_
    return hipGetLastError();
}

template <int WPB>
__global__ __launch_bounds__(64 * WPB) void k_replace(const int32_t* __restrict__ y,
                                                      const double* __restrict__ cooks, int ldn,
                                                      const double* __restrict__ sf,
                                                      const uint8_t* __restrict__ flags,
                                                      const int32_t* __restrict__ gene_idx, int n_sel,
                                                      int N, int cap, int stride, double cutoff,
                                                      int32_t* __restrict__ y_out,
                                                      uint8_t* __restrict__ all_zero, int cooks_ld,
                                                      const int32_t* __restrict__ slot_of) {
    extern __shared__ __attribute__((aligned(16))) double lds[];
    const int w = threadIdx.x >> 6;
    const int k = blockIdx.x * WPB + w;
    if (k >= n_sel) return;
    const int g = gene_idx[k];
    const int32_t* yr = y + (size_t)g * ldn;
    const double* ck = cooks + (size_t)g * (slot_of != nullptr ? (size_t)cooks_ld : (size_t)ldn);
    double* scratch = lds + (size_t)w * stride;
    const double tbm = trimmed_base_mean<DeviceWave>(yr, sf, N, 0.2, scratch, LdsSorter(),
                                                     stride > cap ? (BucketWork*)(scratch + cap) : nullptr);
    int nonzero = 0;
    for (int n = DeviceWave::lane(); n < N; n += 64) {
        int v = yr[n];
        if ((flags[n] & 2) && ck[slot_of != nullptr ? slot_of[n] : n] > cutoff) v = (int)(tbm * sf[n]);
        y_out[(size_t)k * ldn + n] = v;
        nonzero |= (v != 0);
    }
    nonzero = DeviceWave::sumi(nonzero);
    if ((threadIdx.x & 63) == 0) all_zero[k] = (uint8_t)(nonzero == 0);
    if (nonzero == 0)
        for (int n = DeviceWave::lane(); n < N; n += 64) y_out[(size_t)k * ldn + n] = yr[n];
}

template <int WPB>
__global__ __launch_bounds__(64 * WPB) void k_replace_lean(const int32_t* __restrict__ y,
                                                           const double* __restrict__ cooks, int ldn,
                                                           const double* __restrict__ sf,
                                                           const uint8_t* __restrict__ flags,
                                                           const int32_t* __restrict__ gene_idx, int n_sel, int N,
                                                           double cutoff, int32_t* __restrict__ y_out,
                                                           uint8_t* __restrict__ all_zero, int cooks_ld,
                                                           const int32_t* __restrict__ slot_of) {
    __shared__ BucketWork W[WPB];
    const int w = threadIdx.x >> 6;
    const int k = blockIdx.x * WPB + w;
    if (k >= n_sel) return;
    const int g = gene_idx[k];
    const int32_t* yr = y + (size_t)g * ldn;
    const double* ck = cooks + (size_t)g * (slot_of != nullptr ? (size_t)cooks_ld : (size_t)ldn);
    bool failed;
    const double tbm = trimmed_base_mean_lean<DeviceWave>(yr, sf, N, 0.2, W[w], failed);
    int nonzero = 0;
    for (int n = DeviceWave::lane(); n < N; n += 64) {
        int v = yr[n];
        if ((flags[n] & 2) && ck[slot_of != nullptr ? slot_of[n] : n] > cutoff) v = (int)(tbm * sf[n]);
        y_out[(size_t)k * ldn + n] = v;
        nonzero |= (v != 0);
    }
    nonzero = DeviceWave::sumi(nonzero);
    if ((threadIdx.x & 63) == 0) all_zero[k] = (uint8_t)(nonzero == 0);
    if (nonzero == 0)
        for (int n = DeviceWave::lane(); n < N; n += 64) y_out[(size_t)k * ldn + n] = yr[n];
}

hipError_t launch_replace(hipStream_t st, const int32_t* y, const double* cooks, int ldn,
                          const double* sf, const uint8_t* flags, const int32_t* gene_idx, int n_sel,
                          int N, double cutoff, int32_t* y_out, uint8_t* all_zero, int cooks_ld,
                          const int32_t* slot_of) {
    if (n_sel <= 0) return hipSuccess;
    const int cap = next_pow2(N);
    const int stride = cap + trim_work_doubles(N);
    const size_t per_wave = (size_t)stride * sizeof(double);
    static const bool force_lean = getenv("DSQ_REPLACE_LEAN") != nullptr;
    if (per_wave > 160 * 1024 || force_lean) {
        constexpr int WPB = 4;
        hipLaunchKernelGGL(k_replace_lean<WPB>, dim3((n_sel + WPB - 1) / WPB), dim3(64 * WPB), 0, st, y, cooks, ldn, sf,
                           flags, gene_idx, n_sel, N, cutoff, y_out, all_zero, cooks_ld, slot_of);
        return hipGetLastError();
    }
#define DSQ_REPL_LAUNCH(WPB)                                                                         \
    do {                                                                                             \
        if (per_wave * WPB > 48 * 1024) {                                                            \
            (void)hipFuncSetAttribute((const void*)k_replace<WPB>, hipFuncAttributeMaxDynamicSharedMemorySize, \
                                      (int)(per_wave * WPB));                                        \
            (void)hipGetLastError();                                                                 \
        }                                                                                            \
        hipLaunchKernelGGL(k_replace<WPB>, dim3((n_sel + WPB - 1) / WPB), dim3(64 * WPB),            \
                           per_wave * WPB, st, y, cooks, ldn, sf, flags, gene_idx, n_sel, N, cap,    \
                           stride, cutoff, y_out, all_zero, cooks_ld, slot_of);                      \
    } while (0)
    if (per_wave * 4 <= 64 * 1024) DSQ_REPL_LAUNCH(4);
    else if (per_wave * 2 <= 160 * 1024) DSQ_REPL_LAUNCH(2);
    else DSQ_REPL_LAUNCH(1);
#undef DSQ_REPL_LAUNCH
    return hipGetLastError();
}

template <class T>
__global__ __launch_bounds__(256) void k_gather_rows(const T* __restrict__ src, int ld,
                                                     const int32_t* __restrict__ idx, int n_idx,
                                                     int ncols, T* __restrict__ dst,
                                                     const int32_t* __restrict__ n_dev = nullptr) {
    const int k = blockIdx.x;
    if (n_dev != nullptr && k >= *n_dev) return;
    const int g = idx[k];
    for (int c = blockIdx.y * 256 + threadIdx.x; c < ncols; c += gridDim.y * 256)
        dst[(size_t)k * ld + c] = src[(size_t)g * ld + c];
}

hipError_t launch_gather_rows_f64(hipStream_t st, const double* src, int ld, const int32_t* idx,
                                  int n_idx, int ncols, double* dst) {
    if (n_idx <= 0) return hipSuccess;
    const int gx = (ncols + 255) / 256 > 64 ? 64 : (ncols + 255) / 256;
    hipLaunchKernelGGL(k_gather_rows<double>, dim3(n_idx, gx), dim3(256), 0, st, src, ld, idx, n_idx, ncols,
                       dst);
    return hipGetLastError();
}

hipError_t launch_gather_rows_i32(hipStream_t st, const int32_t* src, int ld, const int32_t* idx,
                                  int n_idx, int ncols, int32_t* dst, const int32_t* n_dev) {
    if (n_idx <= 0) return hipSuccess;
    const int gx = (ncols + 255) / 256 > 64 ? 64 : (ncols + 255) / 256;
    hipLaunchKernelGGL(k_gather_rows<int32_t>, dim3(n_idx, gx), dim3(256), 0, st, src, ld, idx, n_idx,
                       ncols, dst, n_dev);
    return hipGetLastError();
}

__global__ void k_trend_eval(const double* __restrict__ nm, int n, double a0, double a1,
                             double* __restrict__ fitted) {
    const int i = blockIdx.x * blockDim.x + threadIdx.x;
    if (i < n) fitted[i] = (a1 == 0.0) ? a0 : a0 + a1 / nm[i];
}

__global__ void k_trend_eval_dev(const double* __restrict__ nm, int n, const double* __restrict__ coef,
                                 double* __restrict__ fitted) {
    const int i = blockIdx.x * blockDim.x + threadIdx.x;
    const double a0 = coef[0], a1 = coef[1];
    if (i < n) fitted[i] = (a1 == 0.0) ? a0 : a0 + a1 / nm[i];
}

__global__ void k_select_disp(double* __restrict__ gw_raw, double* __restrict__ map_raw,
                              const double* __restrict__ fitted, int n, double min_disp, double max_disp,
                              double two_sd, double* __restrict__ disp, uint8_t* __restrict__ outlier) {
    const int i = blockIdx.x * blockDim.x + threadIdx.x;
    if (i >= n) return;
    const double gw = fmin(fmax(gw_raw[i], min_disp), max_disp);
    const double mp = fmin(fmax(map_raw[i], min_disp), max_disp);
    const bool out = log(gw) > log(fitted[i]) + two_sd;
    disp[i] = out ? gw : mp;
    outlier[i] = out ? 1 : 0;
    if (gw_raw[i] == gw_raw[i]) gw_raw[i] = gw;
    if (map_raw[i] == map_raw[i]) map_raw[i] = mp;
}

__global__ void k_select_disp_part(double* __restrict__ gw_raw, double* __restrict__ map_raw,
                                   const double* __restrict__ fitted, int n, double min_disp, double max_disp,
                                   double two_sd, double* __restrict__ disp, uint8_t* __restrict__ outlier,
                                   uint8_t* __restrict__ map_conv, const uint8_t* __restrict__ conv_late,
                                   uint8_t* __restrict__ part, int mode, int ready_limit) {
    const int i = blockIdx.x * blockDim.x + threadIdx.x;
    if (i >= n) return;
    if (mode == 1) {
        const bool ready = map_conv[i] == 1 && i < ready_limit;
        part[i] = ready ? 1 : 0;
        if (!ready) return;
    } else {
        if (part[i] != 0) return;
        if (conv_late != nullptr && conv_late[i] != 0xFF) map_conv[i] = conv_late[i];
    }
    const double gw = fmin(fmax(gw_raw[i], min_disp), max_disp);
    const double mp = fmin(fmax(map_raw[i], min_disp), max_disp);
    const bool out = log(gw) > log(fitted[i]) + two_sd;
// ... 635 lines not shown
```

### pydeseq2_amd/csrc/dsq_launch.h

```cpp
#pragma once
#include <hip/hip_runtime.h>

#include <cstdint>

#include "../../include/deseq_hip.h"
#include "dsq_linalg.h"
#include "dsq_mix.h"

namespace dsq {

constexpr int kWavesPerBlock = 4;
constexpr int kBlock = 64 * kWavesPerBlock;

inline int genes_to_blocks(int G) { return (G + kWavesPerBlock - 1) / kWavesPerBlock; }

inline int current_device_cus() {
    static int cache[64] = {0};
    int dev = 0;
    if (hipGetDevice(&dev) != hipSuccess) return 0;
    if (dev >= 0 && dev < 64 && cache[dev] > 0) return cache[dev];
    hipDeviceProp_t prop;
    if (hipGetDeviceProperties(&prop, dev) != hipSuccess) return 0;
    if (dev >= 0 && dev < 64) cache[dev] = prop.multiProcessorCount;
    return prop.multiProcessorCount;
// ... 95 lines not shown
    const uint16_t* mix_ys;
    const double* mix_mu;
};
constexpr int kAlphaEvalCap = 8;
size_t alpha_resume_bytes(int G);
constexpr int kRowTail = 512;
bool alpha_rows_eligible(int N, int P, int n_cells, bool has_coef, int cr_reg);
hipError_t launch_alpha_rows(hipStream_t st, const int32_t* y, int ldn, int N, const int32_t* list, int n_list,
                             int32_t* queue, const double* coef, const double* sf, const CellDesign& cells, int P,
                             double min_mu, const double* alpha_hat, double min_disp, double max_disp, double prior_var,
                             int cr_reg, int prior_reg, double* alpha, uint8_t* conv, int32_t* nfev, int32_t* grid_count,
                             int32_t* grid_list, double* nll_const, int const_mode, int eval_cap, void* park_state,
                             int32_t* park_count, int32_t* park_list);
hipError_t launch_count_big(hipStream_t st, const int32_t* y, int ldn, int N, int G, int32_t* out);
int alpha_rowsc_tail(int N, int P, int n_cells);
hipError_t launch_alpha_rows_c(hipStream_t st, const int32_t* y, int ldn, int N, const int32_t* list, int n_list,
                               int32_t* queue, const double* coef, const double* cell_mu, const double* sf,
                               const CellDesign& cells, int P, double min_mu, const double* alpha_hat, double min_disp,
                               double max_disp, double prior_var, int prior_reg, double* alpha, uint8_t* conv,
                               int32_t* nfev, int32_t* grid_count, int32_t* grid_list, double* nll_const,
                               int const_mode, int eval_cap, void* park_state, int32_t* park_count,
                               int32_t* park_list);
hipError_t launch_cell_mu(hipStream_t st, const double* beta, const double* Xc, int C, int G, int P, double* cell_mu);
hipError_t launch_mu_from_cells(hipStream_t st, const double* cell_mu, int C, const double* sf, const int32_t* cell_of,
                                int N, const int32_t* list, int n_list, double* dst, int ldn, int32_t* idx_out,
                                const int32_t* n_dev = nullptr);
bool alpha_mix_enabled();
int alpha_mix_launches();
bool alpha_mix_fits(const MixDesign& D);
hipError_t launch_alpha_mix(hipStream_t st, const uint16_t* ys, const double* mu_s, const MixDesign& D, const int32_t* list,
                            int n_list, const int32_t* n_dev, int32_t* queue, const double* alpha_hat, double min_disp,
                            double max_disp, double prior_var, int prior_reg, double* alpha, uint8_t* conv, int32_t* nfev,
                            int32_t* grid_count, int32_t* grid_list, double* nll_const, int const_mode, int eval_cap,
                            int resume, void* park_state, int32_t* park_count, int32_t* park_list);
hipError_t launch_mu_from_beta(hipStream_t st, const double* beta, const double* sf, const double* Xt, int ldx, int N,
                               int P, const int32_t* list, int n_list, double* dst, int ldn, int32_t* idx_out,
                               const int32_t* n_dev = nullptr);
bool alpha_wg_eligible(int N);
hipError_t launch_alpha_wg(hipStream_t st, const int32_t* y, int ldn, int N, const int32_t* list, const int32_t* n_dev,
                           int n_cap, const double* coef, const double* sf, const CellDesign& cells, int P,
                           double min_mu, const double* alpha_hat, double prior_var, int prior_reg, double* alpha,
                           uint8_t* conv, int32_t* nfev, int32_t* grid_count, int32_t* grid_list,
                           const double* nll_const, const void* park_state);
hipError_t launch_alpha_bfgs(hipStream_t st, const int32_t* y, const double* mu, int ldn, const double* Xt, int ldx,
                             int N, int G, int P, const double* alpha_hat, double min_disp, double max_disp,
                             double prior_var, int cr_reg, int prior_reg, double* alpha, uint8_t* conv,
                             int32_t* nfev, int32_t* grid_count, int32_t* grid_list);
hipError_t launch_alpha(hipStream_t st, const int32_t* y, const double* mu, int ldn, const double* Xt,
                        int ldx, int N, int G, int P, const double* alpha_hat, double min_disp,
                        double max_disp, double prior_var, int cr_reg, int prior_reg, double* alpha,
                        uint8_t* conv, int32_t* nfev, int32_t* grid_count, int32_t* grid_list,
                        double* nll_const, int const_mode, const AlphaExtras* extras = nullptr, int32_t* queue = nullptr);
hipError_t launch_alpha_grid(hipStream_t st, const int32_t* y, const double* mu, int ldn, const double* Xt,
                             int ldx, int N, int P, double min_disp, double max_disp, double* alpha,
                             const int32_t* grid_list, int n_grid, double* work, const int32_t* n_dev = nullptr,
                             bool mu_compact = false);
constexpr int kAlphaGridWorkDoubles = 103;

struct IrlsExtras {
    CellDesign cells;
    const double* robust_disp;
    const uint8_t* flags;
    double cutoff;
    double* cooks;
    int cooks_ld;
    double* cooks_tmp;
    uint8_t *any_all, *any_use, *any_use_nr, *few_above;
    const double* ridge;
    const double* contrast;
    double lfc_null;
    int alt;
    double *pvals, *stats, *se;
    int optimizer;
    const int32_t* order;
    const MixDesign* mix;
    void* mix_work;
    size_t mix_work_bytes;
    int32_t* mix_queue;
    const uint16_t* mix_ys;
    const uint8_t* mix_big;
    const uint8_t* part;
    int part_want;
    int part_shared_ready;
};
bool irls_takes_parts(int N, int P, int n_cells, const MixDesign* mix, int full_rank);
bool irls_takes_mix(const MixDesign* mix, int full_rank);
size_t irls_mix_work_bytes(const MixDesign& D, int G, int n_layers);
hipError_t launch_replace(hipStream_t st, const int32_t* y, const double* cooks, int ldn,
                          const double* sf, const uint8_t* flags, const int32_t* gene_idx, int n_sel,
                          int N, double cutoff, int32_t* y_out, uint8_t* all_zero, int cooks_ld,
                          const int32_t* slot_of);
bool irls_takes_rows(int N, int P, int n_cells);
hipError_t launch_irls_order(hipStream_t st, const double* disp, const int32_t* hint_iters, int G, int32_t* order,
                             int32_t* work);
int irls_order_work_ints();
hipError_t launch_irls(hipStream_t st, const int32_t* y, int ldn, const double* sf, const double* lsf,
                       const double* Xt,
                       const double* pinvXt, int ldx, int N, int G, int P, int full_rank,
                       const double* disp, double min_mu, double beta_tol, double min_beta,
                       double max_beta, int maxiter, double* beta, double* mu, double* hat,
                       uint8_t* conv, int32_t* iters, int32_t* fb_count, int32_t* fb_list,
                       const IrlsExtras* extras = nullptr);
hipError_t launch_irls_rescue(hipStream_t st, const int32_t* y, int ldn, const double* sf,
                              const double* lsf, const double* Xt, const double* pinvXt, int ldx, int N, int P,
                              int full_rank, const double* disp, double min_mu, double beta_tol,
                              double min_beta, double max_beta, int maxiter, double* beta, double* mu,
                              double* hat, uint8_t* conv, int32_t* iters, const int32_t* fb_list,
                              int n_fb, const IrlsExtras* extras = nullptr, const int32_t* n_dev = nullptr);

bool irls_is_wide(int P, int n_cells);
bool alpha_is_wide(int P, int n_cells);
bool alpha_needs_mu(int N, int P, int n_cells);

hipError_t launch_widen_u16(hipStream_t st, const uint16_t* src, int32_t* dst, size_t n);
hipError_t launch_transpose_counts(hipStream_t st, const void* src, int count_type, int layout, int N,
                                   int G, int32_t* dst, int ldn, int* bad_flag);
hipError_t launch_transpose_f64(hipStream_t st, const double* src, int layout, int N, int G,
                                double* dst, int ldn);
hipError_t launch_logmeans(hipStream_t st, const int32_t* y, int ldn, int N, int G, double* logmeans,
                           uint8_t* nonzero);
hipError_t launch_size_factors(hipStream_t st, const void* counts_sm, int count_type, int N, int G,
                               const double* logmeans, const uint8_t* gene_mask, double* work,
                               double* sf, int zeros_low = 0);
hipError_t launch_mom(hipStream_t st, const int32_t* y, int ldn, const double* sf, const double* Xt,
                      const double* pinvXt, int ldx, int N, int G, int P, double min_disp,
                      double max_disp, double* normed_mean, double* rough, double* moments,
                      double* mom, double* d_scalar, const double* sf_moments = nullptr);
hipError_t launch_mom_lin_mu(hipStream_t st, const int32_t* y, int ldn, const double* sf, const double* Xt,
                             const double* pinvXt, int ldx, int N, int G, int P, double min_disp, double max_disp,
                             double min_mu, double* normed_mean, double* mom, double* mu, double* d_scalar,
                             double* coef = nullptr);
hipError_t launch_mu_from_coef(hipStream_t st, const double* coef, const double* sf, const double* Xt, int ldx, int N,
                               int P, double min_mu, const int32_t* list, int n_list, double* dst, int ldn,
                               int32_t* idx_out, const int32_t* n_dev = nullptr);
hipError_t launch_irls_layers(hipStream_t st, const int32_t* y, int ldn, const double* sf, const double* Xt, int ldx,
                              int N, int G, int P, const double* disp, const double* beta, double min_mu, double* mu,
                              double* hat);
hipError_t launch_nll_const(hipStream_t st, const int32_t* y, int ldn, int N, int G, const double* disp, double* cst);
hipError_t launch_nll_scaled(hipStream_t st, const int32_t* y, const double* mu, int ldn, int N, int G,
                             const double* disp, const double* scale, const double* cst, double* nll);
hipError_t launch_lin_mu(hipStream_t st, const int32_t* y, int ldn, const double* sf, const double* Xt,
                         const double* pinvXt, int ldx, int N, int G, int P, double min_mu,
                         double* mu);
hipError_t launch_wald(hipStream_t st, const double* mu, int ldn, const double* sf, const double* Xt,
                       int ldx, int N, int G, int P, const double* disp, const double* beta,
                       const double* d_ridge, const double* d_contrast, double lfc_null, int alt,
                       double* pvals, double* stats, double* se);
hipError_t launch_lrt(hipStream_t st, const int32_t* y, int ldn, const double* sf, const double* Xf, int ldf, int Pf,
                      const double* Xr, int ldr, int Pr, int N, int G, const double* disp, const double* beta_f,
                      const double* beta_r, double* stat, double* pval);
hipError_t launch_chisq_sf(hipStream_t st, const double* x, int n, int df, double* out);
hipError_t launch_cooks(hipStream_t st, const int32_t* y, int ldn, const double* sf, const double* mu,
                        const double* hat, const int32_t* cell_offsets, const int32_t* cell_index,
                        int n_cells, int whole, int max_cell, const uint8_t* flags, int N, int G,
                        int P, double cutoff, double* cooks, double* robust_disp, uint8_t* any_all,
                        uint8_t* any_use, uint8_t* any_use_nr, uint8_t* few_above);
hipError_t launch_robust_disp(hipStream_t st, const int32_t* y, int ldn, const double* sf,
                              const int32_t* cell_offsets, const int32_t* cell_index, int n_cells, int whole,
                              int max_cell, int N, int G, double* robust_disp, int min_cell = 0, int32_t* redo = nullptr);
hipError_t launch_gather_rows_f64(hipStream_t st, const double* src, int ld, const int32_t* idx,
                                  int n_idx, int ncols, double* dst);
hipError_t launch_shrink(hipStream_t st, const int32_t* y, int ldn, const double* offset, const double* Xt, int ldx,
                         int N, int G, int P, const double* size, double sigma0, double sigma, int shrink_index,
                         double* beta, double* invh, uint8_t* conv, double* ih_entry = nullptr, int optimizer = 0);
size_t summary_sort_temp_bytes(int n);
hipError_t launch_padj_prepare(hipStream_t st, const double* base_mean, const double* pvalue, int n, double alpha,
                               void* sort_tmp, size_t sort_tmp_bytes, void* work, unsigned long long* sorted_p,
                               int* sorted_idx, unsigned char* bins, double* out200, int* counters);
hipError_t launch_padj_numrej(hipStream_t st, const unsigned long long* sorted_p, const int* sorted_idx,
                              const unsigned char* bins, int n_valid, double alpha, double* out200);
hipError_t launch_padj_finish(hipStream_t st, const unsigned long long* sorted_p, const int* sorted_idx,
                              const unsigned char* bins, int n, int n_valid, int j, int* rank_tmp, double* padj);
hipError_t launch_logmeans_pos(hipStream_t st, const int32_t* y, int ldn, int N, int G, double* logmeans,
                               uint8_t* usable);
// ... 58 lines not shown
```

### pydeseq2_amd/pipeline.py

```python
from __future__ import annotations

import os
import time
import warnings
from dataclasses import dataclass, field

import numpy as np
from scipy.stats import f as f_dist

from . import trend as _trend
from ._design import DesignPack, pad16
from ._lib import ALT, HOOK_FN, I32, I64, SAMPLE_MAJOR, Context, DeviceArray, DsqCells, _PinnedPool, _PinnedSlab

import ctypes as C
import functools

_vp, c_double = C.c_void_p, C.c_double


@dataclass
class DeseqResult:
    size_factors: np.ndarray = None
    normed_means: np.ndarray = None
    non_zero: np.ndarray = None
# ... 58 lines not shown


class _Respeculate(Exception):
    """The pass was enqueued on the previous pass's non-zero mask and the matrix has another one: run it again, in order."""


class _Step:
    """State of one pass of the path: device handles and host scalars the stages hand to each other."""


class _View:

    __slots__ = ("ptr",)

    def __init__(self, ptr):
        self.ptr = ptr


class DeseqPipeline:

    def __init__(self, counts, design_matrix, *, ctx: Context | None = None, device: int = 0, min_mu=0.5,
                 min_disp=1e-8, max_disp=10.0, refit_cooks=True, min_replicates=7, beta_tol=1e-8,
                 fit_type="parametric", keep_cooks=True, size_factors_fit_type="ratio", control_genes=None,
                 irls_maxiter=250):
        self.ctx = ctx if ctx is not None else Context(device)
        counts = np.asarray(counts)
        if counts.ndim != 2:
            raise ValueError("counts must be samples x genes")
        if counts.dtype.kind == "f":
            if np.isnan(counts).any():
                raise ValueError("NaNs are not allowed in the count matrix.")
            if (counts % 1 != 0).any():
                raise ValueError("The count matrix should only contain integers.")
            counts = counts.astype(np.int64)
        elif counts.dtype.kind not in "iu":
            raise ValueError("The count matrix should only contain numbers.")
        if counts.dtype not in (np.int32, np.int64):
            counts = counts.astype(np.int64)
        self.N, self.G = counts.shape
        self.design = DesignPack(design_matrix, min_replicates)
        if self.design.N != self.N:
            raise ValueError("design matrix and counts disagree on the number of samples")
        self.P = self.design.P
        self.min_mu, self.min_disp = float(min_mu), float(min_disp)
        self.max_disp = float(max(max_disp, self.N))
        self.refit_cooks, self.min_replicates = bool(refit_cooks), int(min_replicates)
        self.beta_tol, self.fit_type = float(beta_tol), fit_type
        self.irls_maxiter = int(irls_maxiter)
        self.keep_cooks = keep_cooks
        if size_factors_fit_type not in ("ratio", "poscounts", "iterative"):
            raise ValueError("size_factors_fit_type: 'ratio' (median of ratios), 'poscounts' or 'iterative'")
        self.size_factors_fit_type = size_factors_fit_type
        self._control_mask = None
        if control_genes is not None:
            m = np.zeros(self.G if hasattr(self, "G") else counts.shape[1], dtype=np.uint8)
            m[np.asarray(control_genes)] = 1
            self._control_mask = m
        self.ldn = pad16(self.N)
        ctx_ = self.ctx
        counts = np.ascontiguousarray(counts)
        self._count_type = I32
        self.d_raw = DeviceArray(ctx_, (self.N, self.G), np.int32)
        bad = C.c_int(0)
        ctx_.call("dsq_upload_counts_i32", _vp(counts.ctypes.data), I32 if counts.dtype == np.int32 else I64,
                  C.c_size_t(counts.size), _vp(self.d_raw.ptr), C.byref(bad))
        if bad.value:
            raise ValueError("The count matrix should only contain non-negative integers below 2^31.")
        self.d_y = DeviceArray(ctx_, (self.G, self.N), np.int32, ld=self.ldn)
        ctx_.call("dsq_dev_counts_to_gene_major", _vp(self.d_raw.ptr), I32, SAMPLE_MAJOR, self.N,
                  self.G, _vp(self.d_y.ptr), self.ldn, C.byref(bad))
        D = self.design
        self.d_Xt = DeviceArray.from_host(ctx_, D.Xt)
        self.d_pinv = DeviceArray.from_host(ctx_, D.pinvXt)
        self.d_flags = DeviceArray.from_host(ctx_, D.flags)
        self.d_cell_off = DeviceArray.from_host(ctx_, D.cell_offsets)
        self.d_cell_idx = DeviceArray.from_host(ctx_, D.cell_index)
        self._cells = None
        if D.cell_path and not os.environ.get("DSQ_NO_CELL_PATH"):
            self._d_cell_of = DeviceArray.from_host(ctx_, D.cell_of)
            self._d_Xc = DeviceArray.from_host(ctx_, D.Xc)
            self._d_XXc = DeviceArray.from_host(ctx_, D.XXc)
            self._cells = DsqCells(self._d_cell_of.ptr, self._d_Xc.ptr, self._d_XXc.ptr, int(D.n_design_cells))
        self._row_flags, self._row_lists = None, None
        self._row_mode = 0 if (self._cells is None or os.environ.get("DSQ_NO_ALPHA_ROWS")) else \
            int(ctx_.lib.dsq_alpha_rows_eligible(self.N, self.P, int(D.n_design_cells)))
        if self._row_mode == 1 and not D.linear_mu:
            self._row_mode = 0
        self._mix, self._mix_slots, self._slot_of, self._mix_ys_cache = None, 0, None, None
        if self._row_mode == 0 and not D.linear_mu and not os.environ.get("DSQ_NO_ALPHA_MIX"):
            mp = _vp()
            ctx_.call("dsq_mix_create", _vp(D.X.ctypes.data), self.N, self.P, C.byref(mp))
            if mp.value:
                self._mix, self._row_mode = mp.value, 3
                ns = C.c_int()
                if ctx_.lib.dsq_mix_info(mp, C.byref(ns), None, None) != 0:
                    raise RuntimeError("dsq_mix_info failed")
                self._mix_slots = int(ns.value)
                self._slot_of = np.empty(self.N, dtype=np.int32)
                if ctx_.lib.dsq_mix_slots(mp, _vp(self._slot_of.ctypes.data)) != 0:
                    raise RuntimeError("dsq_mix_slots failed")
        if self._row_mode:
            d_fl = DeviceArray(ctx_, (self.G,), np.int32)
            ctx_.call("dsq_dev_alpha_row_split", _vp(self.d_y.ptr), self.ldn, self.N, self.G, _vp(d_fl.ptr))
            self._row_flags = d_fl.to_host()
            d_fl.free()
        self.keep_layers = False
        self.overlap = not os.environ.get("DSQ_NO_OVERLAP")
        self._robust_early = bool(os.environ.get("DSQ_ROBUST_EARLY"))
        self._robust_late = bool(os.environ.get("DSQ_ROBUST_LATE"))
        mw = os.environ.get("DSQ_MAP_WAIT")
        self._map_waits_side = (self._row_mode == 1) if mw is None else (mw != "0")
        self._robust_split = float(os.environ.get("DSQ_ROBUST_SPLIT", "0.78"))
        lo = os.environ.get("DSQ_LFC_OVERLAP")
        max_work = float(os.environ.get("DSQ_LFC_OVERLAP_MAX_WORK", "1.5e8"))
        auto = self._row_mode == 3 and float(self.G) * self.N <= max_work
        self._lfc_overlap = auto if lo is None else (lo != "0")
        self._lfc_min_genes = int(os.environ.get("DSQ_LFC_OVERLAP_MIN_GENES", "2048"))
        self._lfc_forked = False
        self.lfc_forks = 0
        self._work = None
        self.layers = {}
        self.time_kernels = False
        self.collect_nfev = False
        self.kernel_log = {}
        self._pool_free, self._pool_used = [], []
        self._inflight = []
        self._side_pending = False
        self._pinned = _PinnedPool(ctx_)
        self._replace_buf, self._replace_keep = None, None
        d_lm0, d_nz0 = DeviceArray(ctx_, (self.G,), np.float64), DeviceArray(ctx_, (self.G,), np.uint8)
        ctx_.call("dsq_dev_logmeans", _vp(self.d_y.ptr), self.ldn, self.N, self.G, _vp(d_lm0.ptr), _vp(d_nz0.ptr))
        self._nz_pred = d_nz0.to_host().astype(bool)
        d_lm0.free(); d_nz0.free()
        self._row_lists_for(self._nz_pred)
        self._cooks_cutoff = float(f_dist.ppf(0.99, self.P, self.N - self.P)) if self.N > self.P else float("nan")
        ctx_.sync()

    def _take(self, nbytes):
        nbytes = max(int(nbytes), 8)
        best = None
        for i, (cap, ptr) in enumerate(self._pool_free):
            if cap >= nbytes and (best is None or cap < self._pool_free[best][0]) and cap <= 2 * nbytes + 4096:
                best = i
        if best is not None:
            cap, ptr = self._pool_free.pop(best)
        else:
            cap, ptr = nbytes, self.ctx.malloc(nbytes)
        self._pool_used.append((cap, ptr))
        return ptr

    def _pool_reset(self):
        if getattr(self, "_side_pending", False) or getattr(self, "_lfc_forked", False):
            self.ctx.call("dsq_side_abort")
            self._side_pending = False
            self._lfc_forked = False
        self._pool_free.extend(self._pool_used)
        self._pool_used = []
        self._serial = getattr(self, "_serial", 0) + 1
        if getattr(self, "_inflight", None):
            self.ctx.sync()
        self._inflight = []
        self.layers = {}

    def _pooled(self, shape, dtype, ld=None):
        arr = DeviceArray.__new__(DeviceArray)
        arr.ctx = self.ctx
        arr.shape = tuple(shape)
        arr.dtype = np.dtype(dtype)
        arr.ld = ld if ld is not None else (arr.shape[-1] if len(arr.shape) > 1 else None)
        n = arr.shape[0] * (arr.ld if len(arr.shape) > 1 else 1)
        arr.nbytes = int(n) * arr.dtype.itemsize
        arr.ptr = self._take(arr.nbytes)
        arr.free = lambda: None
        return arr

    def _dvec(self, n, dtype=np.float64):
        return self._pooled((max(int(n), 1),), dtype)

    def _dmat(self, rows, dtype=np.float64):
        return self._pooled((max(int(rows), 1), self.N), dtype, ld=self.ldn)

    def _up(self, arr, dtype=np.float64):
        arr = np.ascontiguousarray(arr, dtype=dtype)
        d = self._pooled(arr.shape if arr.ndim else (1,), arr.dtype)
        if arr.size:
            if arr.nbytes <= 65536:
                hs = self._host_slab(arr.nbytes)
                hs.view(0, arr.size, arr.dtype)[:] = arr.reshape(-1)
                self.ctx.call("dsq_h2d_async", _vp(d.ptr), _vp(hs.ptr), C.c_size_t(arr.nbytes))
                self._inflight.append(hs)
            else:
                self.ctx.h2d(d.ptr, arr)
        return d

    def _down_nonzero(self):
        return self._nz_cache

    def _all_genes_host(self, d_vec, n):
        return self._down(d_vec, n)

    def _down(self, darr, n, dtype=np.float64):
        out = np.empty(int(n), dtype=dtype)
        if n:
            self.ctx.d2h(out, darr.ptr)
        return out

    def _k(self, name, genes, cname, *args):
        if self.time_kernels:
            self.ctx.timer_start()
            self.ctx.call(cname, *args)
            ms = self.ctx.timer_stop()
            self.kernel_log.setdefault(name, []).append((ms, int(genes)))
        else:
            self.ctx.call(cname, *args)
        if cname in ("dsq_dev_alpha_mle", "dsq_dev_alpha_mle2", "dsq_dev_alpha_mle3", "dsq_dev_alpha_mle4"):
            kms, ng = C.c_float(), C.c_int()
            self.ctx.call("dsq_last_alpha_kernel", C.byref(kms), C.byref(ng))
            if kms.value >= 0.0:
                self.kernel_log.setdefault("k_alpha", []).append((float(kms.value), int(genes)))
                self.kernel_log.setdefault("k_alpha_stage", []).append((name, int(genes)))
                self.kernel_log.setdefault("grid_fallback_genes", []).append((float(ng.value), int(genes)))

    _F64 = ("nm", "mom", "gw", "fit", "map", "disp", "p", "stat", "se", "rd")
    _U8 = ("gconv", "mconv", "outl", "lconv", "any_all", "any_use", "any_use_nr", "few_above", "naz")

    def _slab_layout(self, Gs):
        off, o = {}, 0
        for k in self._F64:
            off[k] = o
            o += 8 * Gs
        off["beta"] = o
        o += 8 * Gs * self.P
        n_f64 = o
        for k in self._U8:
            off[k] = o
            o += Gs
        return off, n_f64, ((o + 63) // 64) * 64

    def _dev_slab(self, Gs):
        off, n_f64, total = self._slab_layout(Gs)
        base = self._take(total)
        v = {k: _View(base + o) for k, o in off.items()}
        v["_base"], v["_off"], v["_n_f64"], v["_total"], v["_Gs"] = base, off, n_f64, total, Gs
        return v

    def _host_slab(self, nbytes):
        return self._pinned.take(nbytes)

    def _fetch(self, slab, names=None):
        tok = self._fetch_begin(slab, names)
        self.ctx.sync()
        return self._fetch_end(tok)

    def _fetch_begin(self, slab, names=None):
        Gs, off = slab["_Gs"], slab["_off"]
        width = lambda k: Gs * (8 * self.P if k == "beta" else (8 if k in self._F64 else 1))
        if names is None:
            host, hoff = self._host_slab(slab["_total"]), off
            self.ctx.call("dsq_d2h_async", _vp(host.ptr), _vp(slab["_base"]), C.c_size_t(slab["_total"]))
            names = list(self._F64) + ["beta"] + list(self._U8)
        else:
            hoff, o = {}, 0
            for k in names:
                hoff[k] = o
                o += (width(k) + 63) // 64 * 64
            host = self._host_slab(o)
            for k in names:
                self.ctx.call("dsq_d2h_async", _vp(host.ptr + hoff[k]), _vp(slab["_base"] + off[k]),
                              C.c_size_t(width(k)))
        return host, hoff, names, Gs

    def _fetch_end(self, tok):
        host, hoff, names, Gs = tok
        out = {}
        for k in names:
            if k == "beta":
                out[k] = host.view(hoff[k], Gs * self.P, np.float64).reshape(Gs, self.P)
            elif k in self._F64:
                out[k] = host.view(hoff[k], Gs, np.float64)
            else:
                out[k] = host.view(hoff[k], Gs, np.uint8)
        return out

    def _cells_arg(self):
        return C.byref(self._cells) if self._cells is not None else None

    def _row_lists_for(self, non_zero):
        if self._row_flags is None:
            return None
        c = self._row_lists
        if c is None or not np.array_equal(c[0], non_zero):
            fl = self._row_flags[non_zero]
            rows, waves = np.nonzero(fl >= 0)[0], np.nonzero(fl < 0)[0].astype(np.int32)
            rows = rows[np.argsort(-fl[rows], kind="stable")].astype(np.int32)
            if c is not None:
                c[1].free(); c[3].free()
            d_rows = DeviceArray.from_host(self.ctx, rows if len(rows) else np.zeros(1, np.int32))
            d_waves = DeviceArray.from_host(self.ctx, waves if len(waves) else np.zeros(1, np.int32))
            c = self._row_lists = (non_zero.copy(), d_rows, len(rows), d_waves, len(waves))
        return (c[1], c[2], c[3], c[4]) if c[2] > 0 else None

    def _mix_slots_for(self, d_y, Gs, persistent_key=None):
        if self._mix is None:
            return None
        if persistent_key is not None:
            c = self._mix_ys_cache
            if c is not None and np.array_equal(c[0], persistent_key):
# ... 36 lines not shown
            mh.d_mu = None if (per_cell or from_beta) else self._dmat(Gs)
            self._k("mom", Gs, "dsq_dev_mom", _vp(d_y.ptr), self.ldn, _vp(d_sf.ptr), _vp(self.d_Xt.ptr),
                    _vp(self.d_pinv.ptr), D.ldx, self.N, Gs, self.P, c_double(self.min_disp), c_double(self.max_disp),
                    _vp(S["nm"].ptr), None, None, _vp(S["mom"].ptr))
            d_b, d_c = self._dvec(Gs * self.P), self._dvec(Gs, np.uint8)
            S["_irls_it"] = self._dvec(Gs, np.int32)
            self._mix_bind(mix_slots, genes=Gs)
            self._k("irls_mu", Gs, "dsq_dev_lfc_fit2", _vp(d_y.ptr), self.ldn, _vp(d_sf.ptr), _vp(self.d_Xt.ptr),
                    _vp(self.d_pinv.ptr), D.ldx, self.N, Gs, self.P, int(D.full_rank), _vp(S["mom"].ptr),
                    c_double(self.min_mu), c_double(self.beta_tol), c_double(-30.0), c_double(30.0), self.irls_maxiter,
                    _vp(d_b.ptr), _vp(mh.d_mu.ptr) if mh.d_mu else None, None, _vp(d_c.ptr), _vp(S["_irls_it"].ptr),
                    self._cells_arg(),
                    None, None, c_double(0.0), None, None, None, None, None,
                    None, None, c_double(0.0), 0, None, None, None, _vp(self._mix) if self._mix else None, 0)
            mh.d_beta_fit = d_b
            if from_beta:
                mh.d_beta = d_b
                if mix_slots is not None:
                    mh.d_mu_slots = self._pooled((max(Gs, 1) * self._mix_slots,), np.float64)
                    self.ctx.call("dsq_dev_mix_mu_slots", _vp(self._mix), _vp(d_b.ptr), _vp(d_sf.ptr), Gs,
                                  _vp(mh.d_mu_slots.ptr))
            if per_cell:
                mh.d_cell_mu = self._dvec(Gs * int(D.n_design_cells))
                self.ctx.call("dsq_dev_cell_mu", _vp(d_b.ptr), self._cells_arg(), Gs, self.P, _vp(mh.d_cell_mu.ptr))
        mh.nll_const = self._dvec(Gs)
        if pre_alpha is not None:
            pre_alpha()
        self._alpha_fit("alpha_mle", d_y, mh, Gs, d_sf, S["mom"], 1.0, 0, S["gw"], S["gconv"], 1)
        return mh

    def _alpha_fit(self, name, d_y, mh, Gs, d_sf, d_start, prior_var, prior_reg, d_out, d_conv, const_mode):
        d_nfev = self._dvec(Gs, np.int32) if self.collect_nfev else None
        d_cell_mu = getattr(mh, "d_cell_mu", None)
        d_beta = getattr(mh, "d_beta", None)
        use_coef = mh.d_mu is None and d_cell_mu is None and d_beta is None
        use_cell = d_cell_mu is not None
        mix = self._mix if (self._row_mode == 3 and getattr(mh, "row_lists", None) is not None) else None
        rows = getattr(mh, "row_lists", None) if (mh.d_mu is None or mix) else None
        if mix and rows:
            self._mix_bind(getattr(mh, "mix_slots", None), getattr(mh, "d_mu_slots", None), genes=Gs)
        self._k(name, Gs, "dsq_dev_alpha_mle4", _vp(d_y.ptr), _vp(mh.d_mu.ptr) if mh.d_mu else None, self.ldn,
                _vp(self.d_Xt.ptr), self.design.ldx, self.N, Gs, self.P, _vp(d_start.ptr), c_double(self.min_disp),
                c_double(self.max_disp), c_double(prior_var), 1, int(prior_reg), _vp(d_out.ptr), _vp(d_conv.ptr),
                _vp(d_nfev.ptr) if d_nfev else None, _vp(mh.nll_const.ptr), const_mode, self._cells_arg(),
                _vp(mh.d_coef.ptr) if use_coef else None, _vp(d_sf.ptr) if (use_coef or use_cell or d_beta) else None,
                c_double(self.min_mu), _vp(rows[0].ptr) if rows else None, rows[1] if rows else 0,
                _vp(rows[2].ptr) if rows and rows[3] else None, rows[3] if rows else 0,
                _vp(d_cell_mu.ptr) if use_cell else None, _vp(mix) if (mix and rows) else None,
                _vp(d_beta.ptr) if d_beta else None)
        if d_nfev:
            self.kernel_log.setdefault("nfev", []).append((float(self._down(d_nfev, Gs, np.int32).sum()), Gs))

    def _stage_map(self, d_y, mh, Gs, d_sf, prior_var, squared_logres, S, fork=None):
        if fork is not None:
            self.ctx.call("dsq_alpha_set_late_flags", _vp(fork[1].ptr))
        self._alpha_fit("alpha_map", d_y, mh, Gs, d_sf, S["fit"], prior_var, 1, S["map"], S["mconv"], 2)
        if fork is not None:
            d_part, d_late, forked = fork
            if not forked():
                self.ctx.call("dsq_memset", _vp(d_part.ptr), 0, C.c_size_t(Gs))
            self.ctx.call("dsq_dev_select_dispersions_part", _vp(S["gw"].ptr), _vp(S["map"].ptr), _vp(S["fit"].ptr), Gs,
                          c_double(self.min_disp), c_double(self.max_disp), c_double(squared_logres),
                          _vp(S["disp"].ptr), _vp(S["outl"].ptr), _vp(S["mconv"].ptr), _vp(d_late.ptr), _vp(d_part.ptr),
                          0, 0)
        else:
            self.ctx.call("dsq_dev_select_dispersions", _vp(S["gw"].ptr), _vp(S["map"].ptr), _vp(S["fit"].ptr), Gs,
                          c_double(self.min_disp), c_double(self.max_disp), c_double(squared_logres),
                          _vp(S["disp"].ptr), _vp(S["outl"].ptr))

    def _stage_lfc(self, d_y, Gs, d_sf, S, wald, cooks=None, mix_slots=None, bufs=None, part=None):
        D = self.design
        want = self.keep_layers and cooks is not None
        if bufs is not None:
            d_mu, d_hat = bufs
        else:
            d_mu = self._dmat(Gs) if want else None
            d_hat = self._dmat(Gs) if want else None
        ridge, contrast, lfc_null, alt = wald
        ck = [None, None, c_double(0.0), None, None, None, None, None]
        cooks_ld = 0
        if cooks is not None:
            d_rd, cutoff, d_cooks = cooks
            cooks_ld = self._cooks_ld()
            ck = [_vp(d_rd.ptr), _vp(self.d_flags.ptr), c_double(cutoff), _vp(d_cooks.ptr)] + \
                 [_vp(S[x].ptr) for x in ("any_all", "any_use", "any_use_nr", "few_above")]
        if S.get("_irls_it") is not None:
            self.ctx.call("dsq_irls_order_hint", _vp(S["_irls_it"].ptr), Gs)
        self._mix_bind(mix_slots, genes=Gs)
        if part is not None:
            self.ctx.call("dsq_lfc_set_part", _vp(part[0].ptr), int(part[1]), int(part[2]))
        self._k("lfc_fit", Gs, "dsq_dev_lfc_fit2", _vp(d_y.ptr), self.ldn, _vp(d_sf.ptr), _vp(self.d_Xt.ptr),
                _vp(self.d_pinv.ptr), D.ldx, self.N, Gs, self.P, int(D.full_rank), _vp(S["disp"].ptr),
                c_double(self.min_mu), c_double(self.beta_tol), c_double(-30.0), c_double(30.0), self.irls_maxiter,
                _vp(S["beta"].ptr), _vp(d_mu.ptr) if d_mu else None, _vp(d_hat.ptr) if d_hat else None,
                _vp(S["lconv"].ptr), None, self._cells_arg(), *ck,
                _vp(ridge.ctypes.data), _vp(contrast.ctypes.data), c_double(lfc_null), alt,
                _vp(S["p"].ptr), _vp(S["stat"].ptr), _vp(S["se"].ptr), _vp(self._mix) if self._mix else None, cooks_ld)
        return d_mu, d_hat

    def _replace_rows(self, Gr):
        if self._replace_buf is None or self._replace_buf.shape[0] < Gr:
            if self._replace_buf is not None:
                self.ctx.sync()
                self._replace_buf.free()
            self._replace_buf = DeviceArray(self.ctx, (int(Gr), self.N), np.int32, ld=self.ldn)
        return self._replace_buf

    def _cooks_ld(self):
        if self._mix and self.ctx.lib.dsq_mix_takes_irls(_vp(self._mix), int(self.design.full_rank)):
            return self._mix_slots
        return 0

    def _size_factors(self, d_lm):
        if self._work is None:
            self._work = DeviceArray(self.ctx, (self.ctx.lib.dsq_size_factors_work_doubles(self.N, self.G),),
                                     np.float64)
        d_sf = self._dvec(self.N)
        d_lm, d_mask = self._sf_inputs(d_lm)
        self._k("size_factors", self.G, "dsq_dev_size_factors", _vp(self.d_raw.ptr), self._count_type, self.N,
                self.G, _vp(d_lm.ptr), _vp(d_mask.ptr) if d_mask is not None else None, _vp(self._work.ptr),
                _vp(d_sf.ptr))
        return self._sf_finish(d_sf)

    def _sf_inputs(self, d_lm):
        d_mask = None
        if self.size_factors_fit_type == "poscounts":
            d_lm, d_use = self._dvec(self.G), self._dvec(self.G, np.uint8)
            self.ctx.call("dsq_dev_logmeans_poscounts", _vp(self.d_y.ptr), self.ldn, self.N, self.G, _vp(d_lm.ptr),
                          _vp(d_use.ptr))
            d_mask = d_use
            if self._control_mask is not None:
                d_mask = self._up(self._down(d_use, self.G, np.uint8) & self._control_mask, np.uint8)
        elif self._control_mask is not None:
            d_mask = self._up(self._control_mask, np.uint8)
        return d_lm, d_mask

    def _sf_finish(self, d_sf):
        if self.size_factors_fit_type == "poscounts":
            sf = self._down(d_sf, self.N)
            d_sf = self._up(sf / np.exp(np.mean(np.log(sf))))
        return d_sf

    def _fit_trend(self, Gn):
        d_gw, d_nm = self._last_gw_dev
        return self._run_trend_kernel(d_gw, d_nm, Gn)

    def _run_trend_kernel(self, d_gw, d_nm, n):
        c2, ok, n_outer = (C.c_double * 2)(), C.c_int(0), C.c_int(0)
        d_keep = self._dvec(n, np.uint8)
        self._k("trend_fit", n, "dsq_dev_trend_fit", _vp(d_gw.ptr), _vp(d_nm.ptr), int(n),
                c_double(self.min_disp), c_double(self.max_disp), _vp(d_keep.ptr), c2, C.byref(ok),
                C.byref(n_outer))
        return np.array([c2[0], c2[1]]) if ok.value else None

    def _trend_prior_fused(self, Gn, d_fit):
        d_gw, d_nm = self._last_gw_dev
        c2, ok, n_outer, sq = (C.c_double * 2)(), C.c_int(0), C.c_int(0), C.c_double()
        d_keep = self._dvec(Gn, np.uint8)
        d_work = self._dvec(self.ctx.lib.dsq_prior_mad_work_doubles(int(Gn)))
        self.ctx.call("dsq_dev_trend_prior", _vp(d_gw.ptr), _vp(d_nm.ptr), int(Gn), c_double(self.min_disp),
                      c_double(self.max_disp), _vp(d_keep.ptr), _vp(d_fit.ptr), _vp(d_work.ptr), c2, C.byref(ok),
                      C.byref(n_outer), C.byref(sq))
        if not ok.value:
            return None, None
        return np.array([c2[0], c2[1]]), float(sq.value)

    def _mean_trend(self, Gn):
        d_gw, _ = self._last_gw_dev
        gw = np.clip(self._down(d_gw, Gn), self.min_disp, self.max_disp)
        return _trend.mean_trend(gw, self.min_disp)

    def _prior(self, Gn, d_fit, r):
        d_gw, _ = self._last_gw_dev
        sq = C.c_double()
        d_work = self._dvec(self.ctx.lib.dsq_prior_mad_work_doubles(int(Gn)))
        self._k("prior_mad", Gn, "dsq_dev_prior_mad", _vp(d_gw.ptr), _vp(d_fit.ptr), Gn,
                c_double(self.min_disp), c_double(self.max_disp), _vp(d_work.ptr), C.byref(sq))
        sq = float(sq.value)
        return sq, float(max(sq - _trigamma((self.N - self.P) / 2), 0.25))

    STAGES = ("open", "size_factors", "genewise", "trend", "map", "lfc", "refit", "finish")

    def deseq2(self, contrast=None, lfc_null=0.0, alt_hypothesis=None, profile=False,
               stop_after_trend=False, stop_after_size_factors=False, size_factors=None) -> DeseqResult:
        upto = "size_factors" if stop_after_size_factors else ("trend" if stop_after_trend else "finish")
        while True:
            st = self.begin_step(contrast, lfc_null, alt_hypothesis, profile=profile, size_factors=size_factors,
                                 upto=upto)
            try:
# ... 186 lines not shown
        fused_sq = None
        only_trend = st.stop_at == "trend"
        if self.fit_type == "parametric":
            cls = type(self)
            fused_ok = (cls._trend_prior_fused is not DeseqPipeline._trend_prior_fused
                        or (cls._fit_trend is DeseqPipeline._fit_trend and cls._prior is DeseqPipeline._prior))
            if fused_ok and not (only_trend or self.time_kernels):
                coeffs, fused_sq = self._trend_prior_fused(Gn, S["fit"])
            else:
                coeffs = self._fit_trend(Gn)
            if coeffs is None:
                warnings.warn("The dispersion trend curve fitting did not converge. "
                              "Switching to a mean-based dispersion trend.", UserWarning, stacklevel=3)
        elif self.fit_type != "mean":
            raise NotImplementedError(f"Expected 'parametric' or 'mean' trend curve fit types, received "
                                      f"{self.fit_type}")
        st.coeffs = coeffs
        if coeffs is not None:
            r.trend_coeffs, r.disp_function_type = coeffs, "parametric"
            st.a0, st.a1 = float(coeffs[0]), float(coeffs[1])
        else:
            r.disp_function_type = "mean"
            r.mean_disp = self._mean_trend(Gn)
            st.a0, st.a1 = float(r.mean_disp), 0.0
        if only_trend:
            self.publish(st, ("nm", "mom", "gw", "gconv"))
            return
        if fused_sq is None or coeffs is None:
            self.ctx.call("dsq_dev_trend_eval", _vp(S["nm"].ptr), Gn, c_double(st.a0), c_double(st.a1), _vp(S["fit"].ptr))
        if (N - P) <= 3:
            warnings.warn("As the residual degrees of freedom is less than 3, the distribution of log "
                          "dispersions is especially asymmetric and likely to be poorly estimated by the MAD.",
                          UserWarning, stacklevel=3)
        if fused_sq is not None and coeffs is not None:
            r.squared_logres = fused_sq
            r.prior_disp_var = float(max(fused_sq - _trigamma((N - P) / 2), 0.25))
        else:
            r.squared_logres, r.prior_disp_var = self._prior(Gn, S["fit"], r)
        self._lap(st, "trend_prior")

    def _st_map(self, st):
        ctx, r, S, Gn = self.ctx, st.r, st.S, st.Gn
        if self.overlap and self._map_waits_side and self._side_pending:
            ctx.call("dsq_side_wait")
            self._side_pending = False
        second = st.g_cut < Gn and st.whole
        fork = (self._lfc_overlap and self.overlap and st.whole and not self.time_kernels and not st.profile
                and Gn >= self._lfc_min_genes
                and bool(ctx.lib.dsq_lfc_takes_parts(self.N, self.P, self._cells_arg(), _vp(self._mix) if self._mix else None,
                                                     int(self.design.full_rank))))
        st.lfc_forked = False
        if fork:
            self._lfc_prepare(st)
            st.d_part = self._dvec(Gn, np.uint8)
            st.d_mconv_late = self._dvec(Gn, np.uint8)
            ctx.call("dsq_memset", _vp(S["mconv"].ptr), 0xFF, C.c_size_t(Gn))
            ctx.call("dsq_memset", _vp(st.d_mconv_late.ptr), 0xFF, C.c_size_t(Gn))
            ctx.call("dsq_lfc_prepare", _vp(st.d_sf.ptr), self.N, _vp(st.wald_args[0].ctypes.data),
                     _vp(st.wald_args[1].ctypes.data), self.P)

        def launch():
            if fork:
                self._fork_lfc(st)
            if second or not st.robust_done[1]:
                self._launch_robust(st, 1)

        fit = lambda: self._stage_map(st.d_ynz, st.mh, Gn, st.d_sf, r.prior_disp_var, r.squared_logres, S,
                                      fork=(st.d_part, st.d_mconv_late, lambda: st.lfc_forked) if fork else None)
        if (second or fork) and not self.time_kernels:
            _, fired = self._with_alpha_hook(fit, launch)
        else:
            fit()
            fired = False
        if second and not fired:
            self._launch_robust(st, 1)
        self._lap(st, "MAP")

    def _lfc_prepare(self, st):
        P, Gn = self.P, st.Gn
        st.cutoff = self._cooks_cutoff
        ridge = np.ascontiguousarray(np.diag(np.repeat(1e-6, P)))
        st.wald_args = (ridge, st.contrast, float(np.log(2) * st.lfc_null), ALT[st.alt])
        st.cld = cld = self._cooks_ld()
        st.d_cooks = self._pooled((max(Gn, 1), cld), np.float64, ld=cld) if cld else self._dmat(Gn)

    def _fork_lfc(self, st):
        ctx, r, S, Gn = self.ctx, st.r, st.S, st.Gn
        ctx.call("dsq_lfc_fork_begin")
        self._lfc_forked = True
        try:
            ctx.call("dsq_dev_select_dispersions_part", _vp(S["gw"].ptr), _vp(S["map"].ptr), _vp(S["fit"].ptr), Gn,
                     c_double(self.min_disp), c_double(self.max_disp), c_double(r.squared_logres), _vp(S["disp"].ptr),
                     _vp(S["outl"].ptr), _vp(S["mconv"].ptr), None, _vp(st.d_part.ptr), 1,
                     int(Gn if st.robust_done[1] else st.g_cut))
            st.lfc_bufs = self._stage_lfc(st.d_ynz, Gn, st.d_sf, S, st.wald_args, cooks=(S["rd"], st.cutoff, st.d_cooks),
                                          mix_slots=st.mix_slots, part=(st.d_part, 1, 1))
            ctx.call("dsq_lfc_fork_end")
        except BaseException:
            ctx.call("dsq_side_abort")
            self._lfc_forked = False
            raise
        st.lfc_forked = True
        self.lfc_forks += 1

    def _st_lfc(self, st):
        ctx, D, S, Gn, G = self.ctx, self.design, st.S, st.Gn, self.G
        for part in (0, 1):
            if not st.robust_done[part]:
                self._launch_robust(st, part, side=False)
        forked = getattr(st, "lfc_forked", False)
        if not forked:
            self._lfc_prepare(st)
        cutoff, cld = st.cutoff, st.cld
        if self.overlap and self._side_pending:
            ctx.call("dsq_side_wait")
            self._side_pending = False
        if forked:
            d_mu, d_hat = self._stage_lfc(st.d_ynz, Gn, st.d_sf, S, st.wald_args, cooks=(S["rd"], cutoff, st.d_cooks),
                                          mix_slots=st.mix_slots, bufs=st.lfc_bufs, part=(st.d_part, 0, 2))
            self._lfc_forked = False
        else:
            d_mu, d_hat = self._stage_lfc(st.d_ynz, Gn, st.d_sf, S, st.wald_args, cooks=(S["rd"], cutoff, st.d_cooks),
                                          mix_slots=st.mix_slots)
        st.want_refit = self.refit_cooks and D.replaceable.sum() > 0
        st.flags_tok = self._fetch_begin(S, ["any_all"]) if st.want_refit else None
        st.slab_tok = None
        if st.whole:
            self._begin_block_copy(st)
        if st.all_nz and getattr(self, "_arange_G", None) is None:
            self._arange_G = np.arange(G)
        self.layers = {"nz_idx": self._arange_G if st.all_nz else st.nzi, "mu_LFC": d_mu, "hat_diagonals": d_hat,
                       "cooks": st.d_cooks, "_cooks_ld": cld, "_fit": (st.d_ynz, st.d_sf, S["beta"], S["disp"], Gn)}
        self._lap(st, "LFC_cooks_wald")

    def _begin_block_copy(self, st):
        if self.overlap:
            self.ctx.call("dsq_side_begin")
            self._side_pending = True
            try:
                st.slab_tok = self._fetch_begin(st.S)
            finally:
                self.ctx.call("dsq_side_end")
        else:
            st.slab_tok = self._fetch_begin(st.S)

    def _st_refit(self, st):
        ctx, r, S, Gn, N = self.ctx, st.r, st.S, st.Gn, self.N
        st.replaced_nz = np.zeros(Gn, dtype=bool)
        st.patch = None
        self._replace_keep = None
        if getattr(st, "force_refit", False) and not st.want_refit and self.design.replaceable.sum() > 0:
            st.want_refit, st.flags_tok = True, self._fetch_begin(S, ["any_all"])
        if st.want_refit:
            ctx.sync()
            st.replaced_nz = self._fetch_end(st.flags_tok)["any_all"].astype(bool)
            rp = np.nonzero(st.replaced_nz)[0]
            Gr = len(rp)
            if Gr > 0:
                d_rp = self._up(rp.astype(np.int32), np.int32)
                d_ysub = self._replace_rows(Gr)
                self._replace_keep = {"Gr": Gr, "rp": rp, "nzi": st.nzi, "naz": None}
                S2 = self._dev_slab(Gr)
                d_az = S2["naz"]
                ctx.call("dsq_dev_replace_outliers2", _vp(st.d_ynz.ptr), _vp(st.d_cooks.ptr), self.ldn, _vp(st.d_sf.ptr),
                         _vp(self.d_flags.ptr), _vp(d_rp.ptr), Gr, N, c_double(st.cutoff), _vp(d_ysub.ptr),
                         _vp(d_az.ptr), st.cld, _vp(self._mix) if st.cld else None)
                deferred = not (st.profile or self.time_kernels or self.collect_nfev)
                if deferred:
                    ctx.call("dsq_set_deferred", 1)
                sub_slots = self._mix_slots_for(d_ysub, Gr) if self._mix else None
                try:
                    s_mu = self._stage_genewise(d_ysub, Gr, st.d_sf, S2, mix_slots=sub_slots)
                    ctx.call("dsq_dev_trend_eval", _vp(S2["nm"].ptr), Gr, c_double(st.a0), c_double(st.a1),
                             _vp(S2["fit"].ptr))
                    self._stage_map(d_ysub, s_mu, Gr, st.d_sf, r.prior_disp_var, r.squared_logres, S2)
                    self._stage_lfc(d_ysub, Gr, st.d_sf, S2, st.wald_args, mix_slots=sub_slots)
                finally:
                    if deferred:
                        ctx.call("dsq_set_deferred", 0)
                st.patch = (rp, self._fetch_begin(S2))
        self._lap(st, "refit")

    def _st_finish(self, st):
        ctx, r, G, Gn = self.ctx, st.r, self.G, st.Gn
        if st.slab_tok is None:
            self._begin_block_copy(st)
        if self.overlap:
            ctx.call("dsq_side_wait")
            self._side_pending = False
        ctx.sync()
        H = self._fetch_end(st.slab_tok)
        self._lap(st, "wald")
        all_nz, nzi = st.all_nz, st.nzi

        def full(v, fill=np.nan, dtype=None):
            if all_nz:
                return v if dtype is None else v.astype(dtype)
            out = np.full((G,) + v.shape[1:], fill, dtype=dtype or v.dtype)
            out[nzi] = v
            return out

        replaced_nz = st.replaced_nz
        refitted_nz = np.zeros(Gn, dtype=bool)
        new_zero_nz = np.zeros(Gn, dtype=bool)
        gw = H["gw"]
        nm, fit, disp, beta = H["nm"], H["fit"], H["disp"], H["beta"]
        pv, stt, se = H["p"], H["stat"], H["se"]
        if st.patch is not None:
            rp, h2 = st.patch[0], self._fetch_end(st.patch[1])
            naz = h2["naz"].astype(bool)
            if self._replace_keep is not None:
                self._replace_keep["naz"] = naz.copy()
            new_zero_nz[rp[naz]] = True
            refitted_nz[rp[~naz]] = True
            rf, k = rp[~naz], np.nonzero(~naz)[0]
            nm[rf], fit[rf], disp[rf], beta[rf] = h2["nm"][k], h2["fit"][k], h2["disp"][k], h2["beta"][k]
            gw[rf] = np.clip(h2["gw"][k], self.min_disp, self.max_disp)
            pv[rf], stt[rf], se[rf] = h2["p"][k], h2["stat"][k], h2["se"][k]
            if naz.any():
                zi = rp[naz]
                nm[zi], beta[zi] = 0.0, 0.0
                se[zi], stt[zi], pv[zi] = 0.0, 0.0, 1.0
        r.normed_means = full(nm, fill=0.0)
        r.mom_dispersions = full(H["mom"])
        r.genewise_dispersions = full(gw)
        r.genewise_converged = full(H["gconv"].astype(float))
        r.fitted_dispersions = full(fit) if st.coeffs is not None else np.full(G, r.mean_disp)
        r.MAP_dispersions = full(H["map"])
        r.MAP_converged = full(H["mconv"].astype(float))
        r.outlier_genes = full(H["outl"].view(np.bool_), fill=False)
        r.dispersions = full(disp)
        r.LFC = full(beta)
        r.LFC_converged = full(H["lconv"].astype(float))
        r.replaced = full(replaced_nz, fill=False)
        r.refitted = full(refitted_nz, fill=False)
        r.new_all_zeroes = full(new_zero_nz, fill=False)
        any_use, any_use_nr = H["any_use"].view(np.bool_), H["any_use_nr"].view(np.bool_)
        co_nz = np.where(refitted_nz, any_use_nr, any_use) if (self.refit_cooks and refitted_nz.any()) else any_use
        r.cooks_outlier = full(co_nz & H["few_above"].view(np.bool_), fill=False)
        r.pvalue, r.stat, r.lfcSE = full(pv), full(stt), full(se)
        self._lap(st, "assemble")
        r.timings["total"] = st.t_last - st.t0
        if not self.keep_cooks:
            self.layers = {}
        self._nz_pred = st.non_zero
        st.slab_tok = st.flags_tok = st.patch = None

    def publish(self, st, names):
        r, G = st.r, self.G
# ... 147 lines not shown
            def run(d_y, idx):
                Gs = len(idx)
                d_bf = dev(np.asarray(res.LFC, dtype=np.float64)[idx])
                d_disp = dev(np.asarray(res.dispersions, dtype=np.float64)[idx])
                d_br, d_cv = DeviceArray(ctx, (Gs, Pr), np.float64), DeviceArray(ctx, (Gs,), np.uint8)
                d_out = DeviceArray(ctx, (2 * Gs,), np.float64)
                held.extend([d_br, d_cv, d_out])
                self._k("lrt_reduced_fit", Gs, "dsq_dev_lfc_fit2", _vp(d_y.ptr), self.ldn, _vp(d_sf.ptr), _vp(d_Xr.ptr),
                        _vp(d_pinv.ptr), Dr.ldx, N, Gs, Pr, int(Dr.full_rank), _vp(d_disp.ptr), c_double(self.min_mu),
                        c_double(self.beta_tol), c_double(-30.0), c_double(30.0), self.irls_maxiter, _vp(d_br.ptr), None,
                        None, _vp(d_cv.ptr), None, C.byref(cells) if cells is not None else None,
                        None, None, c_double(0.0), None, None, None, None, None,
                        None, None, c_double(0.0), 0, None, None, None, None, 0)
                self._k("lrt", Gs, "dsq_dev_lrt", _vp(d_y.ptr), self.ldn, _vp(d_sf.ptr), _vp(self.d_Xt.ptr),
                        self.design.ldx, self.P, _vp(d_Xr.ptr), Dr.ldx, Pr, N, Gs, _vp(d_disp.ptr), _vp(d_bf.ptr),
                        _vp(d_br.ptr), _vp(d_out.ptr), _vp(d_out.ptr + 8 * Gs))
                o = d_out.to_host()
                return o[Gs:], o[:Gs], d_br.to_host(), d_cv.to_host().astype(float)

            if Gn > 0:
                if Gn == G:
                    d_y = self.d_y
                else:
                    d_idx = dev(nzi.astype(np.int32))
                    d_y = DeviceArray(ctx, (Gn, N), np.int32, ld=self.ldn)
                    held.append(d_y)
                    ctx.call("dsq_dev_gather_rows_i32", _vp(self.d_y.ptr), self.ldn, _vp(d_idx.ptr), Gn, N, _vp(d_y.ptr))
                pv[nzi], stt[nzi], beta_r[nzi], conv_r[nzi] = run(d_y, nzi)
            if refitted.any():
                rows = np.nonzero(~keep["naz"])[0]
                gidx = (keep["rp"] if keep["nzi"] is None else keep["nzi"][keep["rp"]])[rows]
                if not np.array_equal(np.sort(gidx), np.nonzero(refitted)[0]):
                    raise RuntimeError("lrt(): the kept replaced counts belong to another result")
                d_sel = dev(rows.astype(np.int32))
                d_y2 = DeviceArray(ctx, (len(rows), N), np.int32, ld=self.ldn)
                held.append(d_y2)
                ctx.call("dsq_dev_gather_rows_i32", _vp(self._replace_buf.ptr), self.ldn, _vp(d_sel.ptr), len(rows), N,
                         _vp(d_y2.ptr))
                pv[gidx], stt[gidx], beta_r[gidx], conv_r[gidx] = run(d_y2, gidx)
        finally:
            ctx.sync()
            for a in held:
                a.free()
        z = np.asarray(res.new_all_zeroes, dtype=bool) if res.new_all_zeroes is not None else np.zeros(G, dtype=bool)
        if z.any():
            stt[z], pv[z], beta_r[z] = 0.0, 1.0, 0.0
        return pv, stt, beta_r, conv_r

    def close(self):
        if getattr(self, "_side_pending", False) or getattr(self, "_lfc_forked", False):
            self.ctx.call("dsq_side_abort")
            self._side_pending = False
            self._lfc_forked = False
        for _cap, ptr in self._pool_free + self._pool_used:
            self.ctx.free(ptr)
        self._pool_free, self._pool_used = [], []
        if getattr(self, "_mix_ys_cache", None) is not None:
            self._mix_ys_cache[1].free(); self._mix_ys_cache[2].free()
            self._mix_ys_cache = None
        if getattr(self, "_mix", None):
            self.ctx.lib.dsq_mix_destroy(_vp(self._mix))
            self._mix = None
        if getattr(self, "_replace_buf", None) is not None:
            self._replace_buf.free()
            self._replace_buf, self._replace_keep = None, None
        self._pinned.close()

    def __del__(self):
        try:
            self.close()
        except Exception:
            pass

    def layer(self, name):
        if name == "replace_counts":
            out = self.d_raw.to_host().astype(np.int64)
            k = self._replace_keep
            if k is not None and k["naz"] is not None:
                rows = self.ctx.d2h_rows(self._replace_buf.ptr, k["Gr"], self.N, self.ldn, np.int32)
                rows[k["naz"]] = 0
                out[:, k["rp"] if k["nzi"] is None else k["nzi"][k["rp"]]] = rows.T
            return out
        d = self.layers[name]
        if d is None:
            d_y, d_sf, d_b, d_d, Gn = self.layers["_fit"]
            D = self.design
            self.layers["mu_LFC"], self.layers["hat_diagonals"] = self._dmat(Gn), self._dmat(Gn)
            self.ctx.call("dsq_dev_irls_layers", _vp(d_y.ptr), self.ldn, _vp(d_sf.ptr), _vp(self.d_Xt.ptr), D.ldx,
                          self.N, Gn, self.P, _vp(d_d.ptr), _vp(d_b.ptr), c_double(self.min_mu),
                          _vp(self.layers["mu_LFC"].ptr), _vp(self.layers["hat_diagonals"].ptr))
            d = self.layers[name]
        nzi = self.layers["nz_idx"]
        if name == "cooks" and self.layers.get("_cooks_ld"):
            cld = self.layers["_cooks_ld"]
            rows = self.ctx.d2h_rows(d.ptr, len(nzi), cld, cld)[:, self._slot_of]
        else:
            rows = self.ctx.d2h_rows(d.ptr, len(nzi), self.N, self.ldn)
        out = np.full((self.N, self.G), np.nan)
        out[:, nzi] = rows.T
        return out


def deseq2(counts, design_matrix, contrast=None, *, device=0, ctx=None, lfc_null=0.0, alt_hypothesis=None,
           **kw) -> DeseqResult:
    pipe = DeseqPipeline(counts, design_matrix, ctx=ctx, device=device, **kw)
    return pipe.deseq2(contrast=contrast, lfc_null=lfc_null, alt_hypothesis=alt_hypothesis)
```

Baseline: 10.87 million.

## Compute Cook's distance rows on demand instead of materializing the full matrix

Measured after the change: 10.79 million, median of 2. Within noise of the previous version (-0.7%).

```diff
diff --git a/include/deseq_hip.h b/include/deseq_hip.h
--- a/include/deseq_hip.h
+++ b/include/deseq_hip.h
@@ -220,6 +220,17 @@
 int dsq_dev_replace_outliers2(dsq_ctx* ctx, const int32_t* d_y, const double* d_cooks, int ldn, const double* d_sf,
                               const uint8_t* d_flags, const int32_t* d_gene_idx, int n_sel, int N, double cutoff,
                               int32_t* d_y_out, uint8_t* d_all_zero, int cooks_ld, const dsq_mix* mix);
+int dsq_lfc_set_route(dsq_ctx* ctx, uint8_t* d_route);
+int dsq_lfc_cooks_on_demand(int P, const dsq_cells* cells, const dsq_mix* mix, int full_rank);
+int dsq_dev_cooks_rows(dsq_ctx* ctx, const int32_t* d_y, int ldn, const double* d_sf, const double* d_Xt, int ldx, int N,
+                       int P, const dsq_cells* cells, const double* d_disp, const double* d_beta, const uint8_t* d_route,
+                       const double* d_robust_disp, const uint8_t* d_flags, double cutoff, double min_mu,
+                       const int32_t* d_gene_idx, int n_sel, double* d_out);
+int dsq_dev_replace_outliers_fit(dsq_ctx* ctx, const int32_t* d_y, int ldn, const double* d_sf, const uint8_t* d_flags,
+                                 const int32_t* d_gene_idx, int n_sel, int N, double cutoff, int32_t* d_y_out,
+                                 uint8_t* d_all_zero, const double* d_Xt, int ldx, int P, const dsq_cells* cells,
+                                 const double* d_disp, const double* d_beta, const uint8_t* d_route,
+                                 const double* d_robust_disp, double min_mu);
 int dsq_dev_irls_layers(dsq_ctx* ctx, const int32_t* d_y, int ldn, const double* d_sf, const double* d_Xt, int ldx,
                         int N, int G, int P, const double* d_disp, const double* d_beta, double min_mu, double* d_mu,
                         double* d_hat);
diff --git a/pydeseq2_amd/_lib.py b/pydeseq2_amd/_lib.py
--- a/pydeseq2_amd/_lib.py
+++ b/pydeseq2_amd/_lib.py
@@ -195,6 +195,12 @@
           c_int, c_double, _vp, _vp, _vp, _vp, _vp, _vp)
     proto("dsq_dev_replace_outliers", _vp, _vp, _vp, c_int, _vp, _vp, _vp, c_int, c_int, c_double, _vp, _vp)
     proto("dsq_dev_replace_outliers2", _vp, _vp, _vp, c_int, _vp, _vp, _vp, c_int, c_int, c_double, _vp, _vp, c_int, _vp)
+    proto("dsq_lfc_set_route", _vp, _vp)
+    proto("dsq_lfc_cooks_on_demand", c_int, cells_p, _vp, c_int)
+    proto("dsq_dev_cooks_rows", _vp, _vp, c_int, _vp, _vp, c_int, c_int, c_int, cells_p, _vp, _vp, _vp, _vp, _vp, c_double,
+          c_double, _vp, c_int, _vp)
+    proto("dsq_dev_replace_outliers_fit", _vp, _vp, c_int, _vp, _vp, _vp, c_int, c_int, c_double, _vp, _vp, _vp, c_int,
+          c_int, cells_p, _vp, _vp, _vp, _vp, c_double)
     proto("dsq_dev_wald", _vp, _vp, c_int, _vp, _vp, c_int, c_int, c_int, c_int, _vp, _vp, _vp, _vp,
           c_double, c_int, _vp, _vp, _vp)
     proto("dsq_dev_lrt", _vp, _vp, c_int, _vp, _vp, c_int, c_int, _vp, c_int, c_int, c_int, c_int, _vp, _vp, _vp, _vp, _vp)
@@ -237,6 +243,7 @@
     "dsq_mix_bind", "dsq_mix_bind2", "dsq_dev_mix_counts_to_slots", "dsq_dev_mix_mu_slots",
     "dsq_lfc_fork_begin", "dsq_lfc_fork_end", "dsq_lfc_set_part", "dsq_lfc_takes_parts", "dsq_dev_select_dispersions_part", "dsq_lfc_prepare", "dsq_alpha_set_late_flags",
     "dsq_dev_lrt", "dsq_dev_chisq_sf",
+    "dsq_lfc_set_route", "dsq_lfc_cooks_on_demand", "dsq_dev_cooks_rows", "dsq_dev_replace_outliers_fit",
 ]
 
 
diff --git a/pydeseq2_amd/csrc/dsq_capi_dev.hip b/pydeseq2_amd/csrc/dsq_capi_dev.hip
--- a/pydeseq2_amd/csrc/dsq_capi_dev.hip
+++ b/pydeseq2_amd/csrc/dsq_capi_dev.hip
@@ -548,6 +548,45 @@
     return DSQ_OK;
 }
 
+int dsq_lfc_set_route(dsq_ctx* ctx, uint8_t* d_route) {
+    ctx->lfc_route = d_route;
+    return DSQ_OK;
+}
+
+int dsq_lfc_cooks_on_demand(int P, const dsq_cells* cells, const dsq_mix* mix, int full_rank) {
+    return dsq::irls_cooks_on_demand(P, cells != nullptr ? cells->n_cells : 0, mix != nullptr ? &mix->d : nullptr, full_rank)
+               ? 1 : 0;
+}
+
+int dsq_dev_cooks_rows(dsq_ctx* ctx, const int32_t* d_y, int ldn, const double* d_sf, const double* d_Xt, int ldx, int N,
+                       int P, const dsq_cells* cells, const double* d_disp, const double* d_beta, const uint8_t* d_route,
+                       const double* d_robust_disp, const uint8_t* d_flags, double cutoff, double min_mu,
+                       const int32_t* d_gene_idx, int n_sel, double* d_out) {
+    DSQ_CHECK_ARG(d_y && d_sf && d_Xt && d_disp && d_beta && d_robust_disp && d_flags && d_out, "null argument");
+    DSQ_CHECK_ARG(dsq::irls_cooks_on_demand(P, cells != nullptr ? cells->n_cells : 0, nullptr, 1),
+                  "Cook's rows on demand: a design of at most 4 cells and 4 columns (the others keep their eager layer)");
+    DSQ_HIP(dsq::launch_cooks_rows(ctx->stream, d_y, ldn, d_sf, d_Xt, ldx, N, P, to_cells(cells), d_disp, d_beta, d_route,
+                                   d_robust_disp, d_flags, cutoff, min_mu, d_gene_idx, n_sel, d_out));
+    return DSQ_OK;
+}
+
+int dsq_dev_replace_outliers_fit(dsq_ctx* ctx, const int32_t* d_y, int ldn, const double* d_sf, const uint8_t* d_flags,
+                                 const int32_t* d_gene_idx, int n_sel, int N, double cutoff, int32_t* d_y_out,
+                                 uint8_t* d_all_zero, const double* d_Xt, int ldx, int P, const dsq_cells* cells,
+                                 const double* d_disp, const double* d_beta, const uint8_t* d_route,
+                                 const double* d_robust_disp, double min_mu) {
+    DSQ_CHECK_ARG(d_gene_idx != nullptr, "the genes to replace");
+    if (n_sel <= 0) return DSQ_OK;
+    DSQ_HIP(ensure_ws(ctx, (size_t)n_sel * ldn * sizeof(double)));
+    double* rows = (double*)ctx->d_ws;
+    const int rc = dsq_dev_cooks_rows(ctx, d_y, ldn, d_sf, d_Xt, ldx, N, P, cells, d_disp, d_beta, d_route, d_robust_disp,
+                                      d_flags, cutoff, min_mu, d_gene_idx, n_sel, rows);
+    if (rc != DSQ_OK) return rc;
+    DSQ_HIP(dsq::launch_replace(ctx->stream, d_y, rows, ldn, d_sf, d_flags, d_gene_idx, n_sel, N, cutoff, d_y_out,
+                                d_all_zero, 0, nullptr, true));
+    return DSQ_OK;
+}
+
 int dsq_dev_replace_outliers(dsq_ctx* ctx, const int32_t* d_y, const double* d_cooks, int ldn,
                              const double* d_sf, const uint8_t* d_flags, const int32_t* d_gene_idx,
                              int n_sel, int N, double cutoff, int32_t* d_y_out, uint8_t* d_all_zero) {
diff --git a/pydeseq2_amd/csrc/dsq_capi_internal.h b/pydeseq2_amd/csrc/dsq_capi_internal.h
--- a/pydeseq2_amd/csrc/dsq_capi_internal.h
+++ b/pydeseq2_amd/csrc/dsq_capi_internal.h
@@ -79,6 +79,7 @@
     hipEvent_t ev_lfc_fork = nullptr, ev_lfc_done = nullptr, ev_lfc_part = nullptr;
     const uint8_t* lfc_part = nullptr;
     int lfc_want = 0, lfc_phase = 0;
+    uint8_t* lfc_route = nullptr;
     uint8_t* alpha_conv_late = nullptr;
     int lfc_prepared_N = 0, lfc_prepared_P = 0, lfc_prepared_wald = 0;
     int lfc_pending_G = 0;
@@ -395,6 +396,8 @@
     if (extras != nullptr) ex_local = *extras;
     const dsq::MixDesign* const extras_in_mix = ex_local.mix;
     ex_local.optimizer = optimizer;
+    ex_local.route = ctx->lfc_route;
+    ctx->lfc_route = nullptr;
     DSQ_CHECK_ARG(optimizer == 0 || P <= DSQ_BFGS_MAX_P, "optimizer=\"BFGS\": designs of at most 12 columns");
     extras = &ex_local;
     const uint8_t* const part = ctx->lfc_part;
diff --git a/pydeseq2_amd/csrc/dsq_k_irls.hip b/pydeseq2_amd/csrc/dsq_k_irls.hip
--- a/pydeseq2_amd/csrc/dsq_k_irls.hip
+++ b/pydeseq2_amd/csrc/dsq_k_irls.hip
@@ -115,6 +115,7 @@
         if (iters != nullptr) iters[g] = o.iters;
         if (o.fallback) fb_list[atomicAdd(fb_count, 1)] = g;
         else epilogue_store(E, ex, g);
+        if (ex.route != nullptr) ex.route[g] = (uint8_t)o.fallback;
     }
 #if defined(DSQ_PHASE_TIMING)
     DSQ_PHASE(0);
@@ -381,6 +382,77 @@
         return launch_wide_irls_layers(st, y, ldn, sf, Xt, ldx, N, G, P_, disp, beta, min_mu, mu, hat);
     DSQ_DISPATCH_P(P_, hipLaunchKernelGGL(k_irls_layers<P>, dim3(genes_to_blocks(G)), dim3(kBlock), 0, st, y, ldn, sf,
                                           Xt, ldx, N, G, disp, beta, min_mu, mu, hat))
+    return hipGetLastError();
+}
+
+template <int P, int CS>
+__global__ __launch_bounds__(kBlock) void k_cooks_rows(const int32_t* __restrict__ y, int ldn,
+                                                       const double* __restrict__ sf, const double* __restrict__ Xt,
+                                                       int ldx, int N, CellDesign cells,
+                                                       const double* __restrict__ disp, const double* __restrict__ beta,
+                                                       const uint8_t* __restrict__ route,
+                                                       const double* __restrict__ robust_disp,
+                                                       const uint8_t* __restrict__ flags, double cutoff, double min_mu,
+                                                       const int32_t* __restrict__ gene_idx, int n_sel,
+                                                       double* __restrict__ out) {
+    extern __shared__ __attribute__((aligned(16))) double irls_lds[];
+    constexpr int T = Tri<P>::N;
+    log_tab_fill();
+    double* sXX = irls_lds;
+    double* sXc = sXX + cells.C * T;
+    for (int i = threadIdx.x; i < cells.C * T; i += kBlock) sXX[i] = cells.XX[i];
+    for (int i = threadIdx.x; i < cells.C * P; i += kBlock) sXc[i] = cells.Xc[i];
+    cells.XX = sXX;
+    cells.Xc = sXc;
+    __syncthreads();
+    const int k = blockIdx.x * kWavesPerBlock + (threadIdx.x >> 6);
+    if (k >= n_sel) return;
+    const int g = gene_idx != nullptr ? gene_idx[k] : k;
+    IrlsArgs A;
+    A.y = y + (size_t)g * ldn; A.sf = sf; A.lsf = nullptr; A.Xt = Xt; A.pinvXt = nullptr; A.ldx = ldx; A.N = N;
+    A.disp = disp[g]; A.min_mu = min_mu; A.beta_tol = 0.0; A.min_beta = 0.0; A.max_beta = 0.0; A.maxiter = 0;
+    A.full_rank = false;
+    A.cells = &cells;
+    LfcEpilogue E;
+    E.flags = flags; E.robust_disp = robust_disp[g]; E.cutoff = cutoff;
+    E.cooks_row = out + (size_t)k * ldn;
+    double b[P], M[T], r[P], S;
+#pragma unroll
+    for (int j = 0; j < P; ++j) b[j] = beta[(size_t)g * P + j];
+    if (route != nullptr && route[g] != 0) {
+        irls_sweep<DeviceWave, P>(A, b, 1.0 / A.disp, S, M, r);
+        irls_finish<DeviceWave, P>(A, b, M, nullptr, nullptr, &E);
+    } else {
+        double e_c[CS];
+        irls_sweep_cs<DeviceWave, P, CS>(A, b, 1.0 / A.disp, S, M, r, e_c);
+        irls_finish_cs<DeviceWave, P, CS>(A, b, M, e_c, nullptr, nullptr, &E);
+    }
+}
+
+bool irls_cooks_on_demand(int P_, int n_cells, const MixDesign* mix, int full_rank) {
+    if (mix != nullptr && irls_takes_mix(mix, full_rank)) return false;
+    if (irls_is_wide(P_, n_cells)) return false;
+    return n_cells > 0 && n_cells <= kSmallCells && P_ <= 4;
+}
+
+hipError_t launch_cooks_rows(hipStream_t st, const int32_t* y, int ldn, const double* sf, const double* Xt, int ldx, int N,
+                             int P_, const CellDesign& cells, const double* disp, const double* beta, const uint8_t* route,
+                             const double* robust_disp, const uint8_t* flags, double cutoff, double min_mu,
+                             const int32_t* gene_idx, int n_sel, double* out) {
+    if (n_sel <= 0) return hipSuccess;
+    if (!(cells.C > 0 && cells.C <= kSmallCells && P_ <= 4)) return hipErrorInvalidValue;
+    const dim3 grid(genes_to_blocks(n_sel)), block(kBlock);
+    DSQ_DISPATCH_P(P_, {
+        if constexpr (P <= 4) {
+            const size_t tables = (size_t)cells.C * (Tri<P>::N + P) * sizeof(double);
+            if (cells.C <= 2 && P <= 2)
+                hipLaunchKernelGGL((k_cooks_rows<(P <= 2 ? P : 1), 2>), grid, block, tables, st, y, ldn, sf, Xt, ldx, N,
+                                   cells, disp, beta, route, robust_disp, flags, cutoff, min_mu, gene_idx, n_sel, out);
+            else
+                hipLaunchKernelGGL((k_cooks_rows<P, kSmallCells>), grid, block, tables, st, y, ldn, sf, Xt, ldx, N, cells,
+                                   disp, beta, route, robust_disp, flags, cutoff, min_mu, gene_idx, n_sel, out);
+        }
+    })
     return hipGetLastError();
 }
 
diff --git a/pydeseq2_amd/csrc/dsq_k_stats.hip b/pydeseq2_amd/csrc/dsq_k_stats.hip
--- a/pydeseq2_amd/csrc/dsq_k_stats.hip
+++ b/pydeseq2_amd/csrc/dsq_k_stats.hip
@@ -1155,14 +1155,14 @@
                                                       int N, int cap, int stride, double cutoff,
                                                       int32_t* __restrict__ y_out,
                                                       uint8_t* __restrict__ all_zero, int cooks_ld,
-                                                      const int32_t* __restrict__ slot_of) {
+                                                      const int32_t* __restrict__ slot_of, int rows_by_list) {
     extern __shared__ __attribute__((aligned(16))) double lds[];
     const int w = threadIdx.x >> 6;
     const int k = blockIdx.x * WPB + w;
     if (k >= n_sel) return;
     const int g = gene_idx[k];
     const int32_t* yr = y + (size_t)g * ldn;
-    const double* ck = cooks + (size_t)g * (slot_of != nullptr ? (size_t)cooks_ld : (size_t)ldn);
+    const double* ck = cooks + (size_t)(rows_by_list ? k : g) * (slot_of != nullptr ? (size_t)cooks_ld : (size_t)ldn);
     double* scratch = lds + (size_t)w * stride;
     const double tbm = trimmed_base_mean<DeviceWave>(yr, sf, N, 0.2, scratch, LdsSorter(),
                                                      stride > cap ? (BucketWork*)(scratch + cap) : nullptr);
@@ -1187,14 +1187,14 @@
                                                            const int32_t* __restrict__ gene_idx, int n_sel, int N,
                                                            double cutoff, int32_t* __restrict__ y_out,
                                                            uint8_t* __restrict__ all_zero, int cooks_ld,
-                                                           const int32_t* __restrict__ slot_of) {
+                                                           const int32_t* __restrict__ slot_of, int rows_by_list) {
     __shared__ BucketWork W[WPB];
     const int w = threadIdx.x >> 6;
     const int k = blockIdx.x * WPB + w;
     if (k >= n_sel) return;
     const int g = gene_idx[k];
     const int32_t* yr = y + (size_t)g * ldn;
-    const double* ck = cooks + (size_t)g * (slot_of != nullptr ? (size_t)cooks_ld : (size_t)ldn);
+    const double* ck = cooks + (size_t)(rows_by_list ? k : g) * (slot_of != nullptr ? (size_t)cooks_ld : (size_t)ldn);
     bool failed;
     const double tbm = trimmed_base_mean_lean<DeviceWave>(yr, sf, N, 0.2, W[w], failed);
     int nonzero = 0;
@@ -1213,7 +1213,7 @@
 hipError_t launch_replace(hipStream_t st, const int32_t* y, const double* cooks, int ldn,
                           const double* sf, const uint8_t* flags, const int32_t* gene_idx, int n_sel,
                           int N, double cutoff, int32_t* y_out, uint8_t* all_zero, int cooks_ld,
-                          const int32_t* slot_of) {
+                          const int32_t* slot_of, bool rows_by_list) {
     if (n_sel <= 0) return hipSuccess;
     const int cap = next_pow2(N);
     const int stride = cap + trim_work_doubles(N);
@@ -1222,7 +1222,7 @@
     if (per_wave > 160 * 1024 || force_lean) {
         constexpr int WPB = 4;
         hipLaunchKernelGGL(k_replace_lean<WPB>, dim3((n_sel + WPB - 1) / WPB), dim3(64 * WPB), 0, st, y, cooks, ldn, sf,
-                           flags, gene_idx, n_sel, N, cutoff, y_out, all_zero, cooks_ld, slot_of);
+                           flags, gene_idx, n_sel, N, cutoff, y_out, all_zero, cooks_ld, slot_of, rows_by_list ? 1 : 0);
         return hipGetLastError();
     }
 #define DSQ_REPL_LAUNCH(WPB)                                                                         \
@@ -1234,7 +1234,7 @@
         }                                                                                            \
         hipLaunchKernelGGL(k_replace<WPB>, dim3((n_sel + WPB - 1) / WPB), dim3(64 * WPB),            \
                            per_wave * WPB, st, y, cooks, ldn, sf, flags, gene_idx, n_sel, N, cap,    \
-                           stride, cutoff, y_out, all_zero, cooks_ld, slot_of);                      \
+                           stride, cutoff, y_out, all_zero, cooks_ld, slot_of, rows_by_list ? 1 : 0); \
     } while (0)
     if (per_wave * 4 <= 64 * 1024) DSQ_REPL_LAUNCH(4);
     else if (per_wave * 2 <= 160 * 1024) DSQ_REPL_LAUNCH(2);
diff --git a/pydeseq2_amd/csrc/dsq_launch.h b/pydeseq2_amd/csrc/dsq_launch.h
--- a/pydeseq2_amd/csrc/dsq_launch.h
+++ b/pydeseq2_amd/csrc/dsq_launch.h
@@ -201,6 +201,7 @@
     const uint8_t* part;
     int part_want;
     int part_shared_ready;
+    uint8_t* route;
 };
 bool irls_takes_parts(int N, int P, int n_cells, const MixDesign* mix, int full_rank);
 bool irls_takes_mix(const MixDesign* mix, int full_rank);
@@ -208,7 +209,12 @@
 hipError_t launch_replace(hipStream_t st, const int32_t* y, const double* cooks, int ldn,
                           const double* sf, const uint8_t* flags, const int32_t* gene_idx, int n_sel,
                           int N, double cutoff, int32_t* y_out, uint8_t* all_zero, int cooks_ld,
-                          const int32_t* slot_of);
+                          const int32_t* slot_of, bool rows_by_list = false);
+bool irls_cooks_on_demand(int P, int n_cells, const MixDesign* mix, int full_rank);
+hipError_t launch_cooks_rows(hipStream_t st, const int32_t* y, int ldn, const double* sf, const double* Xt, int ldx, int N,
+                             int P, const CellDesign& cells, const double* disp, const double* beta, const uint8_t* route,
+                             const double* robust_disp, const uint8_t* flags, double cutoff, double min_mu,
+                             const int32_t* gene_idx, int n_sel, double* out);
 bool irls_takes_rows(int N, int P, int n_cells);
 hipError_t launch_irls_order(hipStream_t st, const double* disp, const int32_t* hint_iters, int G, int32_t* order,
                              int32_t* work);
diff --git a/pydeseq2_amd/pipeline.py b/pydeseq2_amd/pipeline.py
--- a/pydeseq2_amd/pipeline.py
+++ b/pydeseq2_amd/pipeline.py
@@ -164,6 +164,7 @@
             self._d_XXc = DeviceArray.from_host(ctx_, D.XXc)
             self._cells = DsqCells(self._d_cell_of.ptr, self._d_Xc.ptr, self._d_XXc.ptr, int(D.n_design_cells))
         self._row_flags, self._row_lists = None, None
+        self._lazy_cooks = None
         self._row_mode = 0 if (self._cells is None or os.environ.get("DSQ_NO_ALPHA_ROWS")) else \
             int(ctx_.lib.dsq_alpha_rows_eligible(self.N, self.P, int(D.n_design_cells)))
         if self._row_mode == 1 and not D.linear_mu:
@@ -304,7 +305,7 @@
                 self.kernel_log.setdefault("grid_fallback_genes", []).append((float(ng.value), int(genes)))
 
     _F64 = ("nm", "mom", "gw", "fit", "map", "disp", "p", "stat", "se", "rd")
-    _U8 = ("gconv", "mconv", "outl", "lconv", "any_all", "any_use", "any_use_nr", "few_above", "naz")
+    _U8 = ("gconv", "mconv", "outl", "lconv", "any_all", "any_use", "any_use_nr", "few_above", "naz", "route")
 
     def _slab_layout(self, Gs):
         off, o = {}, 0
@@ -507,13 +508,15 @@
         if cooks is not None:
             d_rd, cutoff, d_cooks = cooks
             cooks_ld = self._cooks_ld()
-            ck = [_vp(d_rd.ptr), _vp(self.d_flags.ptr), c_double(cutoff), _vp(d_cooks.ptr)] + \
+            ck = [_vp(d_rd.ptr), _vp(self.d_flags.ptr), c_double(cutoff), _vp(d_cooks.ptr) if d_cooks is not None else None] + \
                  [_vp(S[x].ptr) for x in ("any_all", "any_use", "any_use_nr", "few_above")]
         if S.get("_irls_it") is not None:
             self.ctx.call("dsq_irls_order_hint", _vp(S["_irls_it"].ptr), Gs)
         self._mix_bind(mix_slots, genes=Gs)
         if part is not None:
             self.ctx.call("dsq_lfc_set_part", _vp(part[0].ptr), int(part[1]), int(part[2]))
+        if cooks is not None and cooks[2] is None:
+            self.ctx.call("dsq_lfc_set_route", _vp(S["route"].ptr))
         self._k("lfc_fit", Gs, "dsq_dev_lfc_fit2", _vp(d_y.ptr), self.ldn, _vp(d_sf.ptr), _vp(self.d_Xt.ptr),
                 _vp(self.d_pinv.ptr), D.ldx, self.N, Gs, self.P, int(D.full_rank), _vp(S["disp"].ptr),
                 c_double(self.min_mu), c_double(self.beta_tol), c_double(-30.0), c_double(30.0), self.irls_maxiter,
@@ -530,6 +533,13 @@
                 self._replace_buf.free()
             self._replace_buf = DeviceArray(self.ctx, (int(Gr), self.N), np.int32, ld=self.ldn)
         return self._replace_buf
+
+    def _cooks_on_demand(self):
+        if self._lazy_cooks is None:
+            self._lazy_cooks = not os.environ.get("DSQ_EAGER_COOKS") and self._cells is not None and bool(
+                self.ctx.lib.dsq_lfc_cooks_on_demand(self.P, self._cells_arg(), _vp(self._mix) if self._mix else None,
+                                                     int(self.design.full_rank)))
+        return self._lazy_cooks
 
     def _cooks_ld(self):
         if self._mix and self.ctx.lib.dsq_mix_takes_irls(_vp(self._mix), int(self.design.full_rank)):
@@ -882,7 +892,10 @@
         ridge = np.ascontiguousarray(np.diag(np.repeat(1e-6, P)))
         st.wald_args = (ridge, st.contrast, float(np.log(2) * st.lfc_null), ALT[st.alt])
         st.cld = cld = self._cooks_ld()
-        st.d_cooks = self._pooled((max(Gn, 1), cld), np.float64, ld=cld) if cld else self._dmat(Gn)
+        if self._cooks_on_demand():
+            st.d_cooks = None
+        else:
+            st.d_cooks = self._pooled((max(Gn, 1), cld), np.float64, ld=cld) if cld else self._dmat(Gn)
 
     def _fork_lfc(self, st):
         ctx, r, S, Gn = self.ctx, st.r, st.S, st.Gn
@@ -930,7 +943,8 @@
         if st.all_nz and getattr(self, "_arange_G", None) is None:
             self._arange_G = np.arange(G)
         self.layers = {"nz_idx": self._arange_G if st.all_nz else st.nzi, "mu_LFC": d_mu, "hat_diagonals": d_hat,
-                       "cooks": st.d_cooks, "_cooks_ld": cld, "_fit": (st.d_ynz, st.d_sf, S["beta"], S["disp"], Gn)}
+                       "cooks": st.d_cooks, "_cooks_ld": cld, "_fit": (st.d_ynz, st.d_sf, S["beta"], S["disp"], Gn),
+                       "_fit_cooks": (S["rd"], S["route"], cutoff)}
         self._lap(st, "LFC_cooks_wald")
 
     def _begin_block_copy(self, st):
@@ -962,9 +976,16 @@
                 self._replace_keep = {"Gr": Gr, "rp": rp, "nzi": st.nzi, "naz": None}
                 S2 = self._dev_slab(Gr)
                 d_az = S2["naz"]
-                ctx.call("dsq_dev_replace_outliers2", _vp(st.d_ynz.ptr), _vp(st.d_cooks.ptr), self.ldn, _vp(st.d_sf.ptr),
-                         _vp(self.d_flags.ptr), _vp(d_rp.ptr), Gr, N, c_double(st.cutoff), _vp(d_ysub.ptr),
-                         _vp(d_az.ptr), st.cld, _vp(self._mix) if st.cld else None)
+                if st.d_cooks is None:
+                    ctx.call("dsq_dev_replace_outliers_fit", _vp(st.d_ynz.ptr), self.ldn, _vp(st.d_sf.ptr),
+                             _vp(self.d_flags.ptr), _vp(d_rp.ptr), Gr, N, c_double(st.cutoff), _vp(d_ysub.ptr),
+                             _vp(d_az.ptr), _vp(self.d_Xt.ptr), self.design.ldx, self.P, self._cells_arg(),
+                             _vp(S["disp"].ptr), _vp(S["beta"].ptr), _vp(S["route"].ptr), _vp(S["rd"].ptr),
+                             c_double(self.min_mu))
+                else:
+                    ctx.call("dsq_dev_replace_outliers2", _vp(st.d_ynz.ptr), _vp(st.d_cooks.ptr), self.ldn,
+                             _vp(st.d_sf.ptr), _vp(self.d_flags.ptr), _vp(d_rp.ptr), Gr, N, c_double(st.cutoff),
+                             _vp(d_ysub.ptr), _vp(d_az.ptr), st.cld, _vp(self._mix) if st.cld else None)
                 deferred = not (st.profile or self.time_kernels or self.collect_nfev)
                 if deferred:
                     ctx.call("dsq_set_deferred", 1)
@@ -1278,7 +1299,14 @@
                 out[:, k["rp"] if k["nzi"] is None else k["nzi"][k["rp"]]] = rows.T
             return out
         d = self.layers[name]
-        if d is None:
+        if d is None and name == "cooks":
+            d_y, d_sf, d_b, d_d, Gn = self.layers["_fit"]
+            d_rd, d_route, cutoff = self.layers["_fit_cooks"]
+            d = self.layers["cooks"] = self._dmat(Gn)
+            self.ctx.call("dsq_dev_cooks_rows", _vp(d_y.ptr), self.ldn, _vp(d_sf.ptr), _vp(self.d_Xt.ptr), self.design.ldx,
+                          self.N, self.P, self._cells_arg(), _vp(d_d.ptr), _vp(d_b.ptr), _vp(d_route.ptr), _vp(d_rd.ptr),
+                          _vp(self.d_flags.ptr), c_double(cutoff), c_double(self.min_mu), None, Gn, _vp(d.ptr))
+        elif d is None:
             d_y, d_sf, d_b, d_d, Gn = self.layers["_fit"]
             D = self.design
             self.layers["mu_LFC"], self.layers["hat_diagonals"] = self._dmat(Gn), self._dmat(Gn)
```
